# Britefury/cutmix-semisup-seg

Hardware: AMD Instinct MI355X
Metric: train images/sec (student+teacher step) (higher is better)
Workload: dtype bf16; 1 GPU; deeplab2-resnet101 cutmix mean-teacher step, 10x3x321x321, 21 classes (BASELINE configs[1]); per_gpu_batch=10, global_batch=10, classes=21, parallelism=dp1, fuse_batches=True, stream_overlap=True, deterministic_wgrad=False

## Files before the change

cutmix-semisup-seg_amd/_lib.py:

```python
import ctypes as C
import os

import torch

_HERE = os.path.dirname(os.path.abspath(__file__))
LIB_PATH = os.path.join(_HERE, 'csrc', 'libcutmixseg_hip.so')

if not os.path.exists(LIB_PATH):
    raise ImportError('libcutmixseg_hip.so not found at {} -- build it with '
                      '`python cutmix-semisup-seg_amd/build.py` (hipcc, gfx950); there is no CPU fallback'.format(LIB_PATH))

lib = C.CDLL(LIB_PATH)

F32, BF16 = 0, 1
(BN_REDUCE, BN_FINALIZE, BN_APPLY, BN_REDUCE_BWD, BN_BWD_APPLY, BN_COUNT, BN_STATS, BN_FINALIZE_TILES,
 BN_BWD_SUMS_TILES) = range(9)
LABEL_U8, LABEL_I64 = 0, 1
LOSS_IDS = {'var': 0, 'logits_var': 1, 'logits_smoothl1': 2, 'bce': 3, 'kld': 4}
MODE_MIX, MODE_CUT = 0, 1
OPT_CHUNK = 2048
AUG_PARAMS = 24

c_void_p, c_int, c_float, c_size_t = C.c_void_p, C.c_int, C.c_float, C.c_size_t

# ... 78 lines not shown


class StageEntry(C.Structure):
    _fields_ = [('img_off', C.c_longlong), ('lab_off', C.c_longlong), ('hs', c_int), ('ws', c_int)]


class StageDesc(C.Structure):
    _fields_ = [('pool_img', c_void_p), ('pool_labels', c_void_p), ('entries', c_void_p), ('index', c_void_p),
                ('out0', c_void_p), ('out1', c_void_p), ('out_labels', c_void_p), ('out_mask', c_void_p), ('params', c_void_p),
                ('mean', c_float * 3), ('std_', c_float * 3),
                ('n', c_int), ('n_entries', c_int), ('h', c_int), ('w', c_int), ('out_dtype', c_int)]


class PdPatch(C.Structure):
    _fields_ = [('img_off', C.c_longlong), ('hs', c_int), ('ws', c_int), ('cy', c_int), ('cx', c_int)]


class PackItem(C.Structure):
    _fields_ = [('src', c_void_p), ('dst', c_void_p), ('scale', c_void_p),
                ('ntaps', c_int), ('cout', c_int), ('cin', c_int), ('first_block', c_int)]


class WfinishItem(C.Structure):
    _fields_ = [('scratch', c_void_p), ('grad', c_void_p), ('w', c_void_p), ('scale', c_void_p), ('wdot', c_void_p),
                ('ntaps', c_int), ('cout', c_int), ('cin', c_int), ('first_block', c_int)]


_P = C.POINTER


def _proto(name, restype, argtypes):
    fn = getattr(lib, name)
    fn.restype = restype
    fn.argtypes = argtypes
    return fn


PROTOTYPES = {
    'cms_version': (c_int, []),
    'cms_last_error': (C.c_char_p, []),
    'cms_device_info': (c_int, [_P(c_int), C.c_char_p, c_size_t]),
    'cms_boxmask_rasterize': (c_int, [c_void_p, c_int, c_int, c_int, c_int, c_int, c_void_p, c_void_p]),
    'cms_cutmix_paste': (c_int, [c_void_p, c_void_p, c_void_p, c_int, c_void_p, c_int, c_int, c_int, c_int, c_int,
                                 c_int, c_void_p]),
    'cms_cutmix_paste_mask': (c_int, [c_void_p, c_void_p, c_void_p, c_int, c_void_p, c_int, c_int, c_int, c_int,
                                      c_void_p]),
    'cms_consistency_workspace_bytes': (c_size_t, [_P(ConsistencyDesc)]),
    'cms_consistency_fwd': (c_int, [_P(ConsistencyDesc), c_void_p, c_void_p, c_void_p]),
    'cms_consistency_finalize': (c_int, [c_void_p, c_void_p, c_float, c_int, c_float, c_float, c_void_p, c_void_p]),
    'cms_consistency_bwd': (c_int, [_P(ConsistencyDesc), c_void_p, c_void_p, c_void_p]),
    'cms_consistency_fused_supported': (c_int, [_P(ConsistencyDesc)]),
    'cms_consistency_fwd_bwd': (c_int, [_P(ConsistencyDesc), c_float, c_void_p, c_void_p, c_void_p, c_void_p]),
    'cms_scale_by_scalar': (c_int, [c_void_p, C.c_longlong, c_void_p, c_int, c_float, c_void_p]),
    'cms_ict_blend': (c_int, [c_void_p, c_void_p, c_void_p, c_int, c_void_p, c_int, C.c_longlong, c_void_p]),
    'cms_ict_workspace_bytes': (c_size_t, [_P(IctDesc)]),
    'cms_ict_fwd': (c_int, [_P(IctDesc), c_void_p, c_void_p, c_void_p]),
    'cms_ict_bwd': (c_int, [_P(IctDesc), c_void_p, c_void_p, c_void_p, c_void_p]),
    'cms_aug_workspace_bytes': (c_size_t, [_P(AugDesc)]),
    'cms_aug_fwd': (c_int, [_P(AugDesc), c_void_p, c_void_p, c_void_p]),
    'cms_aug_bwd': (c_int, [_P(AugDesc), c_void_p, c_void_p, c_void_p]),
    'cms_ce_workspace_bytes': (c_size_t, [_P(CeDesc)]),
    'cms_ce_fwd': (c_int, [_P(CeDesc), c_void_p, c_void_p, c_void_p]),
    'cms_ce_finalize': (c_int, [c_void_p, c_float, c_void_p, c_void_p]),
    'cms_ce_bwd': (c_int, [_P(CeDesc), c_void_p, c_void_p, c_void_p]),
    'cms_ce_fused_supported': (c_int, [_P(CeDesc)]),
    'cms_ce_fwd_bwd': (c_int, [_P(CeDesc), c_void_p, c_void_p, c_void_p, c_void_p]),
    'cms_upsample_bilinear_fwd': (c_int, [c_void_p, c_void_p, c_int, c_int, c_int, c_int, c_int, c_int, c_int,
                                          c_void_p]),
    'cms_upsample_bilinear_bwd': (c_int, [c_void_p, c_void_p, c_int, c_int, c_int, c_int, c_int, c_int, c_int,
                                          c_void_p]),
    'cms_ema_flat': (c_int, [c_void_p, c_void_p, c_size_t, c_float, c_float, c_void_p, c_void_p]),
    'cms_adam_ema_step': (c_int, [_P(OptimDesc), c_void_p]),
    'cms_sgd_ema_step': (c_int, [_P(OptimDesc), c_void_p]),
    'cms_increment_counter': (c_int, [c_void_p, c_void_p]),
    'cms_bn_fold': (c_int, [c_void_p, c_void_p, c_void_p, c_void_p, c_void_p, c_int, c_float, c_void_p, c_void_p, c_void_p]),
    'cms_argmax_confusion': (c_int, [c_void_p, c_void_p, c_int, c_int, c_int, c_int, c_int, c_int, c_int, c_int,
                                     c_int, c_void_p, c_void_p, c_void_p]),
    'cms_confusion': (c_int, [c_void_p, c_void_p, c_size_t, c_int, c_int, c_void_p, c_void_p]),
    'cms_fill_holes_workspace_bytes': (c_size_t, [c_int, c_int, c_int]),
    'cms_fill_holes': (c_int, [c_void_p, c_void_p, c_void_p, c_int, c_void_p, c_int, c_int, c_int, c_void_p, c_size_t,
                               c_void_p]),
    'cms_conv_igemm': (c_int, [_P(ConvDesc), c_void_p]),
    'cms_conv_igemm_workspace_bytes': (C.c_longlong, []),
    'cms_conv_igemm_route': (c_int, [_P(ConvDesc)]),
    'cms_conv_igemm_stats_tile_rows': (c_int, [_P(ConvDesc)]),
    'cms_frozen_bn_act_bwd': (c_int, [c_void_p, c_void_p, c_void_p, c_void_p, c_int, c_void_p, c_size_t, c_int, c_void_p]),
    'cms_conv_set_trace': (c_int, [c_void_p, c_int]),
    'cms_conv_set_wgrad8': (c_int, [c_int]),
    'cms_loss_set_deterministic': (c_int, [c_int]),
    'cms_conv_wgrad_uses_wgrad8': (c_int, [_P(WgradDesc)]),
    'cms_conv_wgrad': (c_int, [_P(WgradDesc), c_void_p]),
    'cms_conv_wgrad_workspace_bytes': (C.c_longlong, [_P(WgradDesc)]),
    'cms_conv_wgrad_group_kind': (c_int, [_P(WgradDesc)]),
    'cms_conv_wgrad_group_bytes': (C.c_longlong, [c_int]),
    'cms_conv_wgrad_group_pack': (c_int, [_P(WgradDesc), c_int, c_int, c_void_p, C.c_longlong, _P(c_int)]),
    'cms_conv_wgrad_group_run': (c_int, [c_void_p, c_int, c_int, c_int, c_void_p]),
    'cms_conv_pack_transpose': (c_int, [c_void_p, c_int, c_void_p, c_void_p, c_int, c_int, c_int, c_int, c_void_p]),
    'cms_conv_pack_transpose_batch': (c_int, [c_void_p, c_int, c_int, c_int, c_void_p]),
    'cms_conv_pack_transpose_batch64': (c_int, [c_void_p, c_int, c_int, c_void_p]),
    'cms_augment_batch': (c_int, [_P(AugmentDesc), c_void_p]),
    'cms_augment_luma': (c_int, [_P(AugmentDesc), c_void_p, c_void_p]),
    'cms_stage_batch': (c_int, [_P(StageDesc), c_void_p]),
    'cms_stage_luma': (c_int, [_P(StageDesc), c_void_p, c_void_p]),
    'cms_bn_workspace_bytes': (c_size_t, [c_size_t, c_int, c_int]),
    'cms_bn_run': (c_int, [_P(BnOp), c_void_p]),
    'cms_channel_copy': (c_int, [c_void_p, c_size_t, c_void_p, c_size_t, c_size_t, c_int, c_int, c_size_t, c_void_p]),
    'cms_add_n': (c_int, [c_void_p, c_int, c_void_p, c_size_t, c_int, c_void_p]),
    'cms_channel_sum': (c_int, [c_void_p, c_int, c_size_t, c_int, c_void_p, c_void_p]),
    'cms_wgrad_finish_pack': (c_int, [_P(WfinishItem), c_int]),
    'cms_wgrad_finish_run': (c_int, [c_void_p, c_int, c_int, c_void_p]),
    'cms_program_add_channel_sum': (c_int, [c_void_p, c_void_p, c_int, c_size_t, c_int, c_void_p, c_int, c_int]),
    'cms_program_add_wgrad_finish': (c_int, [c_void_p, c_void_p, c_int, c_int, c_int, c_int]),
    'cms_rows_reduce': (c_int, [c_void_p, c_size_t, c_int, c_size_t, c_int, c_int, c_void_p, c_float, c_void_p]),
    'cms_upsample_nhwc': (c_int, [c_void_p, c_void_p, c_size_t, c_int, c_int, c_int, c_int, c_int, c_int, c_int, c_int, c_int,
                                  c_void_p]),
    'cms_aspp_gather_fwd': (c_int, [c_void_p, c_void_p, c_void_p, _P(c_int), _P(c_int), c_int, c_int, c_int, c_int, c_int,
                                    c_int, c_void_p]),
    'cms_aspp_spread_bwd': (c_int, [c_void_p, c_void_p, c_int, _P(c_int), _P(c_int), c_int, c_int, c_int, c_int, c_int,
                                    c_int, c_void_p]),
    'cms_stem_pack_weights': (c_int, [c_void_p, c_int, c_void_p, c_void_p]),
    'cms_stem_out_hw': (c_int, [c_int, c_int, _P(c_int), _P(c_int), _P(c_int), _P(c_int)]),
    'cms_stem_fwd': (c_int, [c_void_p, c_int, c_void_p, c_int, c_void_p, c_void_p, c_void_p, c_int, c_int, c_int,
                             c_void_p]),
    'cms_maxpool3x3s2_fwd': (c_int, [c_void_p, c_void_p, c_void_p, c_int, c_int, c_int, c_int, c_int, c_int, c_void_p]),
    'cms_maxpool3x3s2_relu_bwd': (c_int, [c_void_p, c_void_p, c_void_p, c_void_p, c_int, c_int, c_int, c_int, c_int,
                                          c_int, c_void_p]),
    'cms_stem_wgrad': (c_int, [c_void_p, c_int, c_void_p, c_int, c_void_p, c_void_p, c_int, c_int, c_int, c_void_p]),
    'cms_stem_wgrad_workspace_bytes': (C.c_longlong, [c_int, c_int, c_int, c_int, c_int]),
    'cms_stem_wgrad_ws': (c_int, [c_void_p, c_int, c_void_p, c_int, c_void_p, c_void_p, c_int, c_int, c_int, c_void_p,
                          C.c_longlong, c_void_p]),
    'cms_stem_dgrad': (c_int, [c_void_p, c_int, c_void_p, c_void_p, c_void_p, c_int, c_int, c_int, c_void_p]),
    'cms_program_create': (c_int, [_P(c_void_p)]),
    'cms_program_destroy': (c_int, [c_void_p]),
    'cms_program_add_conv': (c_int, [c_void_p, _P(ConvDesc), c_int, c_int, c_int]),
    'cms_program_add_wgrad': (c_int, [c_void_p, _P(WgradDesc), c_int, c_int, c_int]),
    'cms_program_add_wgrad_group': (c_int, [c_void_p, c_void_p, c_int, c_int, c_int, c_int, c_int]),
    'cms_program_add_memset': (c_int, [c_void_p, c_void_p, c_size_t, c_int, c_int]),
    'cms_program_add_sync': (c_int, [c_void_p, c_int, c_int, c_int]),
    'cms_program_sync_count': (c_int, [c_void_p]),
    'cms_program_set_sync_flags': (c_int, [c_void_p, c_void_p, c_int]),
    'cms_program_add_aspp_gather': (c_int, [c_void_p, c_void_p, c_void_p, c_void_p, _P(c_int), _P(c_int), c_int, c_int,
                                            c_int, c_int, c_int, c_int, c_int, c_int]),
    'cms_program_add_aspp_spread': (c_int, [c_void_p, c_void_p, c_void_p, c_int, _P(c_int), _P(c_int), c_int, c_int, c_int,
                                            c_int, c_int, c_int, c_int, c_int]),
    'cms_program_add_bn': (c_int, [c_void_p, _P(BnOp), c_int, c_int]),
    'cms_program_size': (c_int, [c_void_p]),
    'cms_program_run': (c_int, [c_void_p, c_int, c_int, _P(c_void_p), c_int]),
    'cms_program_run_pair': (c_int, [c_void_p, _P(c_void_p), c_int, c_void_p, _P(c_void_p), c_int]),
    'cms_program_set_timing': (c_int, [c_void_p, c_int]),
    'cms_program_read_timing': (c_int, [c_void_p, _P(C.c_double), _P(C.c_double), _P(C.c_long), _P(C.c_double),
                                        _P(C.c_long)]),
    'cms_conv_igemm_f32': (c_int, [_P(ConvDesc), c_void_p]),
    'cms_conv_wgrad_f32': (c_int, [_P(WgradDesc), c_void_p]),
    'cms_conv_pack_transpose_f32': (c_int, [c_void_p, c_void_p, c_void_p, c_int, c_int, c_int, c_int, c_void_p]),
    'cms_conv_pack_transpose_batch_f32': (c_int, [c_void_p, c_int, c_int, c_void_p]),
    'cms_fft2': (c_int, [c_void_p, c_int, c_int, c_int, c_int, c_void_p, c_void_p, c_void_p]),
    'cms_pd_load_image': (c_int, [c_void_p, _P(StageEntry), c_int, c_int, c_int, c_int, c_void_p, c_void_p, c_void_p]),
    'cms_pd_load_patches': (c_int, [c_void_p, c_void_p, c_int, c_int, c_int, c_int, c_int, c_void_p, c_void_p]),
    'cms_pd_patch_sqdiff': (c_int, [c_void_p, c_void_p, c_void_p, c_int, c_int, c_int, c_void_p, c_void_p]),
    'cms_pd_spectrum_product': (c_int, [c_void_p, c_void_p, c_int, c_int, c_int, c_void_p, c_void_p]),
    'cms_pd_finish': (c_int, [c_void_p, c_void_p, c_void_p, c_int, c_int, c_int, c_int, c_int, c_void_p, c_void_p, c_void_p,
                              c_void_p]),
    'cms_select_workspace_bytes': (c_size_t, [c_int]),
    'cms_select_k_smallest': (c_int, [c_void_p, c_void_p, c_void_p, c_void_p, c_int, c_int, C.c_longlong, c_int, c_void_p, c_void_p,
                                      c_void_p, c_size_t, c_void_p]),
    'cms_pd_box_sum': (c_int, [c_void_p, c_int, c_int, c_int, c_int, c_int, c_void_p, c_void_p, c_void_p]),
    'cms_pd_neighbour_workspace_bytes': (c_size_t, [c_int, c_int, c_int, c_int]),
    'cms_pd_neighbour_maps': (c_int, [c_void_p, _P(StageEntry), c_int, c_int, c_void_p, c_void_p, c_void_p]),
    'cms_downsample_image_u8': (c_int, [c_void_p, c_int, c_int, c_int, c_int, c_void_p, c_void_p]),
    'cms_downsample_labels_u8': (c_int, [c_void_p, c_int, c_int, c_int, c_int, c_void_p, c_void_p]),
    'cms_cowmask_workspace_bytes': (c_size_t, [c_int, c_int, c_int]),
    'cms_cowmask': (c_int, [c_void_p, c_void_p, c_void_p, c_int, c_int, c_int, c_int, c_void_p, c_void_p, c_void_p, c_size_t,
                            c_void_p]),
}

fn = {}
for _name, (_res, _args) in PROTOTYPES.items():
    fn[_name] = _proto(_name, _res, _args)


class CmsError(RuntimeError):
    pass


def check(rc, what=''):
    if rc == 0:
        return
    msg = fn['cms_last_error']().decode(errors='replace')
    if rc == -1:
        raise ValueError('{}: {}'.format(what or 'cutmixseg', msg))
    raise CmsError('{} failed (code {}): {}'.format(what or 'cutmixseg', rc, msg))


def version():
    return fn['cms_version']()
```

cutmix-semisup-seg_amd/backbone_hip.py:

```python
import os
import torch

from . import ops
from .arena import ensure_arena


def executors_of(module):
    exs = getattr(module, '_hip_executors', None)
    if exs:
        return list(exs.values())
    ex = getattr(module, '_hip_executor', None)
    return [] if ex is None else [ex]


class _Conv(object):
    __slots__ = ('wkey', 'bn', 'taps', 'ntaps', 'neg_taps', 'stride', 'cin', 'cout', 'scale', 'bias', 'wT', 'ksize',
                 'pad', 'dil', 'wdot', 'dbeta', 'wT_raw')

    def __init__(self, wkey, bn, conv):
        self.wkey, self.bn = wkey, bn
        kh, kw = conv.kernel_size
        self.ksize, self.pad, self.dil = kh, conv.padding[0], conv.dilation[0]
        self.taps = ops.conv_taps(kh, kw, conv.dilation[0], conv.padding[0])
        self.neg_taps = [(-dy, -dx) for dy, dx in self.taps]
# ... 13 lines not shown
        self._init_common(net, dtype)
        self.num_classes = net.num_classes
        self._add_blocks('', [getattr(net, 'layer{}'.format(li)) for li in range(1, 5)])
        self.stem_wkey, self.stem_bn, self.stem_ceil = 'conv1.weight', 'bn1', True
        self.stem_w147 = None
        self._stem_version = -1
        head = net.layer5.conv2d_list
        self.aspp_keys = ['layer5.conv2d_list.0', 'layer5.conv2d_list.1']
        self.aspp_taps = []
        for i in range(2):
            self.aspp_taps += ops.conv_taps(3, 3, head[i].dilation[0], head[i].padding[0])
        self.aspp_neg_taps = [(-dy, -dx) for dy, dx in self.aspp_taps]
        dev = self.arena.device
        C = self.num_classes
        if C > 32:
            raise NotImplementedError('ASPP head kernel is specialised for <= 32 classes')
        self.aspp_zc = (18 * C + 127) // 128 * 128
        self.aspp_wall = torch.zeros(1, self.aspp_zc, 2048, dtype=self.dtype, device=dev)
        self.aspp_wallT = torch.zeros(1, 2048, self.aspp_zc, dtype=self.dtype, device=dev)
        self._aspp_version = -1
        self.aspp_bias = torch.zeros(C, dtype=torch.float32, device=dev)

    def _init_common(self, net, dtype=torch.bfloat16):
        if dtype not in (torch.bfloat16, torch.float32):
            raise TypeError('executor dtype must be torch.bfloat16 or torch.float32')
        self.net = net
        self.dtype = dtype
        self.trainable = any(p.requires_grad for p in net.parameters())
        self.bn_trainable = any(p.requires_grad for m in net.modules() if 'BatchNorm' in type(m).__name__
                                for p in m.parameters())
        self.arena = ensure_arena(net, with_grad=self.trainable, with_bf16=(dtype == torch.bfloat16))
        self.blocks = []
        self._layer_first = []
        self._affine_ready = False
        self._bn_idx = None
        self._side = None
        self._pack_plan = None
        self._pack_plan_bn = None
        self._wT_raw_version = -1
        self._bn_modules = {}
        self._stem_param = None
        self._sentinel = None
        self._seen_shapes = {}
        self._wscratch_buf = None
        self._wfinish_pending = []
        self._wfinish_ok = {}
        self._pending_keep = None
        self.grad_hook = None
        self.data_grad_only = False
        self.overlap_wgrad = True
        self.wgrad_streams = 2 if os.environ.get('CMS_WGRAD8', '1') != '0' else 1
        self.defer_wgrad_join = False
        self._pending_join = None
        self._sides = []
        self.conv_tile = 0
        self.tile_rules = {}
        self._wT_version = -1
        self.version = 0
        self.use_programs = True
        self._programs = {}
        self._generation = 0
        self.issued = dict(flops=0.0, conv_launches=0, conv_bytes=0.0, head_launches=0, head_bytes=0.0, head_bytes_alg=0.0, floor_s=0.0)
        net.register_load_state_dict_post_hook(lambda module, incompatible: self.invalidate())

    def _add_blocks(self, prefix, layers):
        for li, layer in enumerate(layers):
            self._layer_first.append(len(self.blocks))
            for bi, blk in enumerate(layer):
                pre = '{}layer{}.{}'.format(prefix, li + 1, bi)
                b = _Block()
                b.c1 = _Conv(pre + '.conv1.weight', pre + '.bn1', blk.conv1)
                b.c2 = _Conv(pre + '.conv2.weight', pre + '.bn2', blk.conv2)
                b.c3 = _Conv(pre + '.conv3.weight', pre + '.bn3', blk.conv3)
                b.cd = None
                if blk.downsample is not None:
                    b.cd = _Conv(pre + '.downsample.0.weight', pre + '.downsample.1', blk.downsample[0])
                self.blocks.append(b)

    def invalidate(self):
        self.arena.refresh_bf16()
        self._affine_ready = False
        self.version += 1

    def weights_changed(self, bn_too=False):
        self.version += 1
        if bn_too or self.bn_trainable:
            self._affine_ready = False

    def block_grad_offsets(self):
        return [self.arena.by_key[b.c1.wkey].offset for b in self.blocks]

    def layer_first_blocks(self):
        return list(self._layer_first)

    def _all_convs(self):
        for b in self.blocks:
            for c in (b.c1, b.c2, b.c3, b.cd):
                if c is not None:
                    yield c

    def _build_affine_tables(self):
        a = self.arena
        idx = {k: [] for k in ('weight', 'bias', 'running_mean', 'running_var')}
        off = 0
        spans = []
        for c in self._all_convs():
# ... 193 lines not shown
            ops.bn_op('sums_tiles', c=C, dtype=self.dtype, n_pixels=npix, groups=G, tile_rows=tile_stats['tile_rows'],
                      ws=tile_stats['tile_sums'], sums=sums)
        else:
            ops.bn_op('reduce_bwd', c=C, dtype=self.dtype, n_pixels=npix, groups=G, x=u, dy=dy, mean=mean, rstd=rstd, sums=sums,
                      ws=ws, mask_bits=bits)
        grp = self._dist_group()
        world = ops._world(grp)
        if world > 1:
            ops.host_call(lambda t=sums, g_=grp: ops._allreduce_sum(t, g_))
        du = torch.empty_like(u)
        dres = torch.empty_like(u) if want_res else None
        ops.bn_op('bwd_apply', c=C, dtype=self.dtype, n_pixels=npix, groups=G, count=(npix // G) * world, x=u, dy=dy, dx=du, dres=dres,
                  mask_bits=bits, mean=mean, rstd=rstd, gamma=self.arena.view(c.bn + '.weight'), sums=sums)
        return du, dres

    def _fwd_block_bn(self, st, bi):
        b, cur = self.blocks[bi], st['cur']
        save, G = st['saved'] is not None, st.get('groups', 1)
        a1, s1 = self._fwd_unit_bn(cur, b.c1, True, save=save, groups=G)
        a2, s2 = self._fwd_unit_bn(a1, b.c2, True, save=save, groups=G)
        sd = None
        if b.cd is None:
            res = cur
        else:
            res, sd = self._fwd_unit_bn(cur, b.cd, False, save=save, groups=G)
        out, s3 = self._fwd_unit_bn(a2, b.c3, True, res=res, save=save, groups=G)
        st['cur'] = out
        if st['saved'] is not None:
            st['saved'].append((cur, a1, a2, s1, s2, s3, sd))

    def _refresh_backward_weights_bn(self):
        if self._pack_plan_bn is None:
            triples = []
            for c in self._all_convs():
                w = self._w(c)
                c.wT_raw = torch.empty((w.shape[0], w.shape[2], w.shape[1]), dtype=self.dtype, device=w.device)
                triples.append((w, c.wT_raw, None))
            triples.append((self.aspp_wall, self.aspp_wallT, None))
            self._pack_plan_bn = ops.PackTransposePlan(triples)
        self._pack_plan_bn.run()

    def _dgrad_raw(self, du, c, res=None, in_hw=None, res_bits=None, bstats=None):
        n, ho, wo, _ = du.shape
        if c.stride == 1:
            return ops.conv_igemm(du, c.wT_raw, c.neg_taps, res=res, mode=1, tile=self._tile(c.cin), mask_bits=res_bits,
                                  mask_gates_res=res_bits is not None, stats=bstats)
        assert res_bits is None and bstats is None
        return ops.conv_igemm(du, c.wT_raw, c.neg_taps, res=res, mode=1, out_hw=(ho, wo), out_stride=c.stride,
                              out_full_hw=in_hw, tile=self._tile(c.cin))

    def _wgrad_raw(self, du, x, c):
        ops.conv_wgrad(du, x, c.taps, self.arena.packed(c.wkey, self.arena.grad), stride=c.stride, wg_target=self._wg_target())

    def _backward_chain_bn(self, saved, dlg, want_w, sides, hook, box=None):
        x4 = saved[-1]
        main = torch.cuda.current_stream()
        d = ops.aspp_spread_bwd(dlg, self.aspp_taps, self.aspp_zc, self.dtype)
        dwall = None
        if want_w:
            dwall = torch.empty((1, self.aspp_zc, 2048), dtype=torch.float32, device=d.device)
            ops.memset_zero(dwall)
            ops.conv_wgrad(d, x4, [(0, 0)], dwall)
            if box is not None:
                box['dwall'] = dwall
        pend = self._bstats(saved[len(self.blocks) - 1][5])
        dOut = ops.conv_igemm(d, self.aspp_wallT, [(0, 0)], mode=1, stats=pend)
        keep = []
        closes = set(self.bucket_starts())
        for bi in range(len(self.blocks) - 1, -1, -1):
            b = self.blocks[bi]
            xin, a1, a2, s1, s2, s3, sd = saved[bi]
            in_hw = (xin.shape[1], xin.shape[2])
            bits3 = s3[1] if (b.cd is not None or (b.c1.stride == 1 and self.dtype == torch.bfloat16)) else None
            du3, dres = self._bwd_unit_bn(dOut, s3, b.c3, bits3 is None, tile_stats=pend)
            da2 = self._dgrad_raw(du3, b.c3)
            du2, _ = self._bwd_unit_bn(da2, s2, b.c2, False)
            da1 = self._dgrad_raw(du2, b.c2)
            du1, _ = self._bwd_unit_bn(da1, s1, b.c1, False)
            dud = None
            if b.cd is not None:
                dud, _ = self._bwd_unit_bn(dres if bits3 is None else dOut, sd, b.cd, False, dy_bits=bits3)
            if want_w:
                self._issue_wgrads(self._block_jobs(b, du3, du2, dud, du1, xin, a1, a2), sides, main, keep, bi in closes,
                                   wgrad=self._wgrad_raw)
                with torch.cuda.stream(sides[0] if sides else main):
                    hook(bi)
            pend = self._bstats(saved[bi - 1][5]) if (bi > 0 and b.c1.stride == 1) else None
            if b.cd is None and bits3 is not None:
                dOut = self._dgrad_raw(du1, b.c1, res=dOut, in_hw=in_hw, res_bits=bits3, bstats=pend)
            else:
                dx = dres if b.cd is None else self._dgrad_raw(dud, b.cd, in_hw=in_hw)
                dOut = self._dgrad_raw(du1, b.c1, res=dx, in_hw=in_hw, bstats=pend)
        if not self.defer_wgrad_join:
            for sd_ in sides:
                ops.stream_wait(main, sd_)
        self._retire_keep(keep)
        return dOut, dwall

    def _stem_prepare(self):
        if not self._affine_ready:
            self._refresh_affine()
        if self._stem_version != self.version:
            self.stem_w147 = ops.stem_pack_weights(self.arena.packed(self.stem_wkey, self._wbuf()), out=self.stem_w147)
            self._stem_version = self.version

    def stem(self, x):
        if self._stem_param is None:
            self._stem_param = dict(self.net.named_parameters())[self.stem_wkey]
        save = (torch.is_grad_enabled() and (self.trainable or x.requires_grad)) if self.use_programs else None
        return _StemFn.apply(x.contiguous(), self._stem_param, self, save)
# ... 130 lines not shown
    def _wscratch(self):
        if self._wscratch_buf is None:
            self._wscratch_buf = torch.zeros_like(self.arena.grad)
        return self._wscratch_buf

    def _wfinish_takes(self, du, x, c):
        if self.dtype != torch.bfloat16 or ops.deterministic_wgrad():
            return False
        key = (c.wkey, tuple(du.shape), tuple(x.shape))
        hit = self._wfinish_ok.get(key)
        if hit is None:
            hit = self._wfinish_ok[key] = bool(ops.conv_wgrad(du, x, c.taps, self.arena.packed(c.wkey, self._wscratch()),
                                                              stride=c.stride, scale=None, wg_target=self._wg_target(),
                                                              query_kernel=True))
        return hit

    def _wfinish_flush(self):
        pend = self._wfinish_pending
        if not pend:
            return
        a = self.arena
        ops.wgrad_finish([(a.packed(c.wkey, self._wscratch()), a.packed(c.wkey, a.grad), self._w(c), c.scale, c.wdot) for c in pend])
        del pend[:]

    def _wg_target(self):
        if not self.overlap_wgrad:
            return 0
        return 56 if self.wgrad_streams >= 2 else 112

    def _dgrad(self, du, c, res=None, mask=None, in_hw=None):
        n, ho, wo, _ = du.shape
        mb = getattr(mask, '_cms_relu_bits', None) if mask is not None else None
        if mb is not None:
            mask = None
        if c.stride == 1:
            return ops.conv_igemm(du, c.wT, c.neg_taps, res=res, mode=1, mask_src=mask, tile=self._tile(c.cin), mask_bits=mb)
        return ops.conv_igemm(du, c.wT, c.neg_taps, res=res, mode=1, mask_src=mask, out_hw=(ho, wo),
                              out_stride=c.stride, out_full_hw=in_hw, tile=self._tile(c.cin), mask_bits=mb)

    def _grad_sentinel(self):
        if self._sentinel is None:
            self._sentinel = dict(self.net.named_parameters())[self.blocks[-1].c3.wkey]
        return self._sentinel

    def _want_w(self):
        data_only = self.data_grad_only or getattr(self.net, '_data_grad_only', False)
        return self.trainable and not data_only and self.arena.grad is not None

    def _refresh_for_backward(self):
        if self._wT_version != self.version or self.blocks[0].c1.wT is None:
            self._refresh_backward_weights()
            self._wT_version = self.version

    def _head_bias_grads(self, dlogits, want_w, side=None):
        if want_w:
            if side is not None:
                side.wait_stream(torch.cuda.current_stream())
                dlogits.record_stream(side)
            with torch.cuda.stream(side if side is not None else torch.cuda.current_stream()):
                db = dlogits.sum(dim=(0, 2, 3))
                for k in self.aspp_keys:
                    self.arena.view(k + '.bias', self.arena.grad).add_(db)

    def _head_weight_grads(self, dwall, side=None):
        C = self.num_classes
        a = self.arena
        with torch.cuda.stream(side if side is not None else torch.cuda.current_stream()):
            for i, k in enumerate(self.aspp_keys):
                a.packed(k + '.weight', a.grad).add_(dwall[0, 9 * C * i:9 * C * (i + 1)].view(9, C, 2048))

    def _finish_head(self, dwall, side):
        self._head_weight_grads(dwall, side)
        if side is not None and not self.defer_wgrad_join:
            torch.cuda.current_stream().wait_stream(side)

    def bucket_starts(self):
        l2, l3, l4 = self._layer_first[1], self._layer_first[2], self._layer_first[3]
        return sorted(set([0, l2, l3, (l3 + l4 + 1) // 2, l4]))

    def _backward_chain(self, saved, dlg, want_w, sides, hook, box=None):
        x4 = saved[-1]
        main = torch.cuda.current_stream()
        d = ops.aspp_spread_bwd(dlg, self.aspp_taps, self.aspp_zc, self.dtype)
        dwall = None
        keep = []
        if want_w:
            dwall = torch.empty((1, self.aspp_zc, 2048), dtype=torch.float32, device=d.device)
            hs = sides[0] if sides else None
            if hs is not None:
                ops.stream_wait(hs, main)
                keep.append((d, dwall))
            with torch.cuda.stream(hs if hs is not None else main):
                ops.memset_zero(dwall)
                ops.conv_wgrad(d, x4, [(0, 0)], dwall)
            if box is not None:
                box['dwall'] = dwall
        x4b = getattr(x4, '_cms_relu_bits', None)
        dC = ops.conv_igemm(d, self.aspp_wallT, [(0, 0)], mode=1, mask_src=None if x4b is not None else x4, mask_bits=x4b)
        capture = getattr(self, 'debug_capture', None)
        closes = set(self.bucket_starts())
        for bi in range(len(self.blocks) - 1, -1, -1):
            if capture is not None:
                capture[bi] = dC
            b = self.blocks[bi]
            xin, a1, a2 = saved[bi]
            in_hw = (xin.shape[1], xin.shape[2])
            dU2 = self._dgrad(dC, b.c3, mask=a2)
            dU1 = self._dgrad(dU2, b.c2, mask=a1)
            if want_w:
                self._issue_wgrads(self._block_jobs(b, dC, dU2, dC, dU1, xin, a1, a2), sides, main, keep, bi in closes)
                with torch.cuda.stream(sides[0] if sides else main):
                    hook(bi)
            dres = dC if b.cd is None else self._dgrad(dC, b.cd, in_hw=in_hw)
            dC = self._dgrad(dU1, b.c1, res=dres, mask=None if bi == 0 else xin, in_hw=in_hw)
        if not self.defer_wgrad_join:
            for sd in sides:
                ops.stream_wait(main, sd)
        self._retire_keep(keep)
        return dC, dwall

    def backward(self, token, dlogits):
        bn = (token[0].bn if self.use_programs and isinstance(token, tuple) and isinstance(token[0], ops.Program)
              else len(token[0]) == 7)
        chain = self._backward_chain_bn if bn else self._backward_chain
        if bn:
            if self._wT_raw_version != self.version or self.blocks[0].c1.wT_raw is None:
                self._refresh_aspp_fwd()
                self._refresh_backward_weights_bn()
                self._wT_raw_version = self.version
        else:
            self._refresh_for_backward()
        want_w = self._want_w()
        if want_w and self._grad_sentinel().grad is None:
            self.arena.ensure_grads_attached()
        n, _, h, w = dlogits.shape
        main = torch.cuda.current_stream()
        sides = self._side_streams(self.wgrad_streams) if (self.overlap_wgrad and want_w) else []
        hside = sides[0] if (sides and not bn) else None
        if not self.use_programs:
            if self.defer_wgrad_join and sides:
                self._pending_join = list(sides)
            self._head_bias_grads(dlogits, want_w, hside)
            box = {}

            def hook(bi):
                if 'done' not in box and box.get('dwall') is not None:
                    self._head_weight_grads(box['dwall'])
                    box['done'] = True
                if self.grad_hook is not None:
                    self.grad_hook(bi)
            dx, dwall = chain(token, dlogits, want_w, sides, hook, box)
            if dwall is not None and 'done' not in box:
                self._finish_head(dwall, hside)
            return dx
        fprog, gen = token
        if fprog.generation != gen:
            raise RuntimeError('the activations of this forward pass were overwritten by a later forward pass of the '
                               'same shape through the same executor (programs keep ONE set of buffers per shape): '
                               'run backward before the next forward, or set executor.use_programs = False')
        key = (want_w, len(sides), bool(self.defer_wgrad_join))
        if self.defer_wgrad_join and sides:
            self._pending_join = list(sides)
        prog = fprog.bwd.get(key)
        if prog is None:
            prog = ops.Program()
            dlg = torch.empty(tuple(dlogits.shape), dtype=torch.float32, device=dlogits.device)
            streams = [main] + sides
            with ops.recording(prog, streams):
                dx, dwall = chain(fprog.saved, dlg, want_w, sides, prog.mark)
            prog.dlg, prog.dx, prog.dwall = dlg, dx, dwall
            fprog.bwd[key] = prog
        prog.dlg.copy_(dlogits)
        self._head_bias_grads(dlogits, want_w, hside)
        streams = [main] + sides
        if self.grad_hook is None or not want_w:
            prog.run(streams)
            if prog.dwall is not None:
                self._finish_head(prog.dwall, hside)
        else:
            first = 0
            hook_stream = sides[0] if sides else main
            head_done = False
            wanted = getattr(self.grad_hook, 'blocks', None)
            for idx, bi in prog.marks:
                if wanted is not None and bi not in wanted:
                    continue
                prog.run(streams, first, idx)
                first = idx
                with torch.cuda.stream(hook_stream):
                    if not head_done and prog.dwall is not None:
                        self._head_weight_grads(prog.dwall)
                        head_done = True
                    self.grad_hook(bi)
            prog.run(streams, first, -1)
            if prog.dwall is not None and not head_done:
                self._finish_head(prog.dwall, hside)
        self._account(prog)
        return prog.dx.clone()

    def _retire_keep(self, keep):
        if keep and self.defer_wgrad_join and ops._REC is None:
            self._pending_keep = (self._pending_keep or []) + [keep]

    def join_wgrad(self):
        sides, self._pending_join = self._pending_join, None
        if sides:
            main = torch.cuda.current_stream()
            for sd in sides:
                main.wait_stream(sd)
        self._pending_keep = None

    @staticmethod
    def _block_jobs(b, d3, d2, dd, d1, xin, a1, a2):
        return [(d3, a2, b.c3), (d2, a1, b.c2)] + ([(dd, xin, b.cd)] if b.cd is not None else []) + [(d1, xin, b.c1)]

    def _issue_wgrads(self, jobs, sides, main, keep, closes, first=0, wgrad=None):
        wgrad = wgrad or self._wgrad
        for sd in sides:
            ops.stream_wait(sd, main)
        if sides:
            keep.append(jobs)
        for ji, (du_, x_, c_) in enumerate(jobs, first):
            with torch.cuda.stream(sides[ji % len(sides)] if sides else main):
                wgrad(du_, x_, c_)
        if closes:
            for sd in sides[1:]:
# ... 479 lines not shown
        logits, token = executor.forward(x_nhwc, save=need_grad)
        ctx.executor = executor
        ctx.saved_acts = token
        return logits

    @staticmethod
    def backward(ctx, dlogits):
        dx = ctx.executor.backward(ctx.saved_acts, dlogits.contiguous().float())
        ctx.saved_acts = None
        return dx, None, None


class _BodyPairFn(torch.autograd.Function):

    @staticmethod
    def forward(ctx, x_stu, x_tea, ex_stu, ex_tea, side, need_grad):
        if ex_stu.use_programs and ex_tea.use_programs:
            main = torch.cuda.current_stream()
            ps = ex_stu.forward_program(x_stu.shape, need_grad)
            ex_stu._prepare_forward()
            if x_stu.data_ptr() != ps.x_in.data_ptr():
                ps.x_in.copy_(x_stu)
            with torch.cuda.stream(side):
                pt = ex_tea.forward_program(x_tea.shape, False)
                ex_tea._prepare_forward()
                if x_tea.data_ptr() != pt.x_in.data_ptr():
                    pt.x_in.copy_(x_tea)
            if ps.host_ops or pt.host_ops:
                with torch.cuda.stream(side):
                    pt.run([side])
                ps.run([main])
            else:
                ops.run_pair(ps, [main], pt, [side])
            ex_stu._stamp(ps)
            ex_tea._stamp(pt)
            logits_s = ps.logits.clone()
            with torch.cuda.stream(side):
                logits_t = pt.logits.clone()
            saved = (ps, ps.generation) if need_grad else None
        else:
            st_s = ex_stu.fwd_begin(x_stu, need_grad)
            with torch.cuda.stream(side):
                st_t = ex_tea.fwd_begin(x_tea, False)
            for bi in range(len(ex_stu.blocks)):
                ex_stu.fwd_block(st_s, bi)
                with torch.cuda.stream(side):
                    ex_tea.fwd_block(st_t, bi)
            logits_s, saved = ex_stu.fwd_end(st_s)
            with torch.cuda.stream(side):
                logits_t, _ = ex_tea.fwd_end(st_t)
        ctx.executor = ex_stu
        ctx.saved_acts = saved
        ctx.mark_non_differentiable(logits_t)
        return logits_s, logits_t

    @staticmethod
    def backward(ctx, dlogits, _unused):
        dx = ctx.executor.backward(ctx.saved_acts, dlogits.contiguous().float())
        ctx.saved_acts = None
        return dx, None, None, None, None, None


def run_body_pair(ex_stu, x_stu, ex_tea, x_tea, side):
    if len(ex_stu.blocks) != len(ex_tea.blocks):
        raise ValueError('student and teacher bodies differ')
    need_grad = torch.is_grad_enabled() and ex_stu.trainable
    if need_grad and not x_stu.requires_grad:
        x_stu = x_stu.detach().requires_grad_(True)
    return _BodyPairFn.apply(x_stu, x_tea, ex_stu, ex_tea, side, need_grad)


def run_body(executor, x_nhwc):
    need_grad = torch.is_grad_enabled() and (executor.trainable or x_nhwc.requires_grad)
    if need_grad and not x_nhwc.requires_grad:
        x_nhwc = x_nhwc.detach().requires_grad_(True)
    return _BodyFn.apply(x_nhwc, executor, need_grad)
```

cutmix-semisup-seg_amd/csrc/aspp.hip:

```cpp
#include "common.hpp"

namespace cms {

struct AsppTaps {
    int n_taps;
    short dy[CMS_CONV_MAX_TAPS], dx[CMS_CONV_MAX_TAPS];
};

__device__ __forceinline__ void taps_to_lds(const AsppTaps& tp, short* sdy, short* sdx) {
#pragma unroll
    for (int i = 0; i < CMS_CONV_MAX_TAPS; ++i)
        if ((int)threadIdx.x == i) {
            sdy[i] = tp.dy[i];
            sdx[i] = tp.dx[i];
        }
    __syncthreads();
}

__global__ __launch_bounds__(256) void aspp_gather_fwd_kernel(const float* __restrict__ z, const float* __restrict__ bias,
                                                              float* __restrict__ logits, AsppTaps tp, int N, int C, int ZC,
                                                              int H, int W) {
    __shared__ short sdy[CMS_CONV_MAX_TAPS], sdx[CMS_CONV_MAX_TAPS];
    taps_to_lds(tp, sdy, sdx);
    const int n_taps = tp.n_taps;
    const size_t total = (size_t)N * C * H * W;
    for (size_t i = (size_t)blockIdx.x * blockDim.x + threadIdx.x; i < total; i += (size_t)gridDim.x * blockDim.x) {
        const unsigned ii = (unsigned)i;
        const int x = (int)(ii % (unsigned)W);
        unsigned t = ii / (unsigned)W;
        const int y = (int)(t % (unsigned)H); t /= (unsigned)H;
        const int c = (int)(t % (unsigned)C);
        const int n = (int)(t / (unsigned)C);
        float acc = bias ? bias[c] : 0.0f;
        const float* zn = z + ((size_t)n * ZC + c) * H * W;
        const size_t tap_stride = (size_t)C * H * W;
        for (int k = 0; k < n_taps; ++k) {
            const int yy = y + sdy[k], xx = x + sdx[k];
            if ((unsigned)yy < (unsigned)H && (unsigned)xx < (unsigned)W) acc += zn[(size_t)k * tap_stride + (size_t)yy * W + xx];
        }
        logits[i] = acc;
    }
}

template <class T>
__global__ __launch_bounds__(256) void aspp_spread_bwd_kernel(const float* __restrict__ dl, T* __restrict__ d, AsppTaps tp,
                                                              int N, int C, int ZC, int H, int W) {
    __shared__ short sdy[CMS_CONV_MAX_TAPS], sdx[CMS_CONV_MAX_TAPS];
    taps_to_lds(tp, sdy, sdx);
    const int n_taps = tp.n_taps;
    const unsigned zc8 = (unsigned)ZC / 8u;
    const size_t total = (size_t)N * H * W * zc8;
    const size_t plane = (size_t)H * W;
    for (size_t i = (size_t)blockIdx.x * blockDim.x + threadIdx.x; i < total; i += (size_t)gridDim.x * blockDim.x) {
        const unsigned ii = (unsigned)i;
        const unsigned ch = ii % zc8;
        unsigned t = ii / zc8;
        const int x = (int)(t % (unsigned)W); t /= (unsigned)W;
        const int y = (int)(t % (unsigned)H);
        const int n = (int)(t / (unsigned)H);
        const float* dn = dl + (size_t)n * C * plane;
        float v[8];
        int k = (int)((ch * 8u) / (unsigned)C), c = (int)(ch * 8u) - k * C;
#pragma unroll
        for (int e = 0; e < 8; ++e) {
            float val = 0.0f;
            if (k < n_taps) {
                const int yy = y - sdy[k], xx = x - sdx[k];
                if ((unsigned)yy < (unsigned)H && (unsigned)xx < (unsigned)W) val = dn[(size_t)c * plane + (size_t)yy * W + xx];
            }
            v[e] = val;
            if (++c == C) { c = 0; ++k; }
        }
        if constexpr (sizeof(T) == 4) {
            float4* o = reinterpret_cast<float4*>(d + i * 8);
            o[0] = float4{v[0], v[1], v[2], v[3]};
            o[1] = float4{v[4], v[5], v[6], v[7]};
        } else {
            uint4 o;
            o.x = (uint32_t)f32_to_bf16(v[0]) | ((uint32_t)f32_to_bf16(v[1]) << 16);
            o.y = (uint32_t)f32_to_bf16(v[2]) | ((uint32_t)f32_to_bf16(v[3]) << 16);
            o.z = (uint32_t)f32_to_bf16(v[4]) | ((uint32_t)f32_to_bf16(v[5]) << 16);
            o.w = (uint32_t)f32_to_bf16(v[6]) | ((uint32_t)f32_to_bf16(v[7]) << 16);
            *reinterpret_cast<uint4*>(d + i * 8) = o;
        }
    }
}

}

using namespace cms;

static int fill_taps(AsppTaps& tp, const int* dy, const int* dx, int n_taps) {
    CMS_REQUIRE(dy && dx && n_taps > 0 && n_taps <= CMS_CONV_MAX_TAPS, "aspp: 1..%d taps", CMS_CONV_MAX_TAPS);
    tp.n_taps = n_taps;
    for (int i = 0; i < CMS_CONV_MAX_TAPS; ++i) {
        tp.dy[i] = (short)(i < n_taps ? dy[i] : 0);
        tp.dx[i] = (short)(i < n_taps ? dx[i] : 0);
    }
    return CMS_OK;
}

extern "C" int cms_aspp_gather_fwd(const float* z, const float* bias, float* logits, const int* tap_dy, const int* tap_dx,
                                   int n_taps, int n, int c, int zc, int h, int w, void* stream) {
    CMS_REQUIRE(z && logits, "aspp_gather_fwd: NULL pointer");
    CMS_REQUIRE(n > 0 && c > 0 && h > 0 && w > 0 && zc >= n_taps * c, "aspp_gather_fwd: bad geometry (zc >= taps * classes)");
    AsppTaps tp;
    const int rc = fill_taps(tp, tap_dy, tap_dx, n_taps);
    if (rc) return rc;
    const size_t total = (size_t)n * c * h * w;
    CMS_REQUIRE(total < (1ull << 32), "aspp_gather_fwd: more than 2^32 logits");
    hipLaunchKernelGGL(aspp_gather_fwd_kernel, dim3(grid_for(total, 256, 256 * 16)), dim3(256), 0, (hipStream_t)stream, z, bias,
                       logits, tp, n, c, zc, h, w);
    return launch_status("cms_aspp_gather_fwd");
}

extern "C" int cms_aspp_spread_bwd(const float* dlogits, void* d_nhwc, int d_dtype, const int* tap_dy, const int* tap_dx,
                                   int n_taps, int n, int c, int zc, int h, int w, void* stream) {
    CMS_REQUIRE(dlogits && d_nhwc, "aspp_spread_bwd: NULL pointer");
    CMS_REQUIRE(d_dtype == CMS_F32 || d_dtype == CMS_BF16, "aspp_spread_bwd: bad dtype");
    CMS_REQUIRE(n > 0 && c > 0 && h > 0 && w > 0 && zc >= n_taps * c, "aspp_spread_bwd: bad geometry (zc >= taps * classes)");
    AsppTaps tp;
    const int rc = fill_taps(tp, tap_dy, tap_dx, n_taps);
    if (rc) return rc;
    CMS_REQUIRE(zc % 8 == 0, "aspp_spread_bwd: the stacked tap x class axis (%d) must be a multiple of 8", zc);
    const size_t total = (size_t)n * h * w * (zc / 8);
    CMS_REQUIRE(total < (1ull << 32), "aspp_spread_bwd: more than 2^32 chunks");
    hipStream_t s = (hipStream_t)stream;
    if (d_dtype == CMS_F32)
        hipLaunchKernelGGL(aspp_spread_bwd_kernel<float>, dim3(grid_for(total, 256, 256 * 16)), dim3(256), 0, s, dlogits,
                           (float*)d_nhwc, tp, n, c, zc, h, w);
    else
        hipLaunchKernelGGL(aspp_spread_bwd_kernel<uint16_t>, dim3(grid_for(total, 256, 256 * 16)), dim3(256), 0, s, dlogits,
                           (uint16_t*)d_nhwc, tp, n, c, zc, h, w);
    return launch_status("cms_aspp_spread_bwd");
}
```

cutmix-semisup-seg_amd/csrc/loss_tiles.hpp:

```cpp
#pragma once
#include <algorithm>
#include <cstdlib>
#include "common.hpp"

namespace cms {

template <bool IDENT>
struct Gather {
    const float* base;
    size_t plane;
    int w_in;
    Tap ty, tx;
    size_t off;
    __device__ __forceinline__ float operator()(int c) const {
        if (IDENT) return base[c * plane + off];
        return bilin_gather(base + c * plane, w_in, ty, tx);
    }
};

template <int CT>
struct RegVec {
    float v[CT > 0 ? CT : 1];
    __device__ __forceinline__ float operator()(int c) const { return v[c]; }
};
// ... 123 lines not shown
    const int ty_i = b % tiles_y;
    ScatterTile t;
    t.n = b / tiles_y;
    t.x0 = tx_i * TILE_W;
    t.y0 = ty_i * FWD_TILE_H;
    t.tw = min(TILE_W, g.W - t.x0);
    t.th = min(FWD_TILE_H, g.H - t.y0);
    return t;
}

template <bool UNROLL, class Stage, class Pixel>
__device__ __forceinline__ void fwd_tile_walk(const Geo& g, float* smem, Stage stage, Pixel pixel) {
    const ScatterTile t = fwd_tile(g);
    const Patch p = tile_patch(g, t.x0, t.y0, t.tw, t.th);
    stage(t.n, p, smem);
    __syncthreads();
    const int col = threadIdx.x & (TILE_W - 1);
    auto rows = [&](int rr) {
        const int row = (threadIdx.x >> 6) + rr * 4;
        if (col < t.tw && row < t.th) {
            const int y = t.y0 + row, x = t.x0 + col;
            Tap ty = bilin_tap(y, g.sy, g.h, g.align != 0), tx = bilin_tap(x, g.sx, g.w, g.align != 0);
            rebase(ty, tx, p);
            pixel(t.n, y, x, ty, tx, p);
        }
    };
    if (UNROLL) {
#pragma unroll
        for (int rr = 0; rr < FWD_TILE_H / 4; ++rr) rows(rr);
    } else {
#pragma unroll 1
        for (int rr = 0; rr < FWD_TILE_H / 4; ++rr) rows(rr);
    }
}

template <class F>
__device__ __forceinline__ void pixel_walk(const Geo& g, F f) {
    const size_t P = (size_t)g.n * g.H * g.W;
    for (size_t idx = (size_t)blockIdx.x * blockDim.x + threadIdx.x; idx < P; idx += (size_t)gridDim.x * blockDim.x) {
        const int x = (int)(idx % g.W);
        const size_t t = idx / g.W;
        const int y = (int)(t % g.H);
        const int n = (int)(t / g.H);
        f(idx, n, y, x);
    }
}

template <int K>
__device__ __forceinline__ void store_partials(float (&acc)[K], float* red, float* __restrict__ partials) {
    block_sum<K>(acc, red);
    if (threadIdx.x == 0) {
#pragma unroll
        for (int k = 0; k < K; ++k) partials[blockIdx.x * K + k] = acc[k];
    }
}

template <int K>
__global__ __launch_bounds__(256) void reduce_partials_kernel(const float* __restrict__ partials, int nblocks,
                                                              double* __restrict__ out, double extra, int extra_slot) {
    __shared__ double sm[K][256];
    double loc[K];
#pragma unroll
    for (int k = 0; k < K; ++k) loc[k] = 0.0;
    for (int i = threadIdx.x; i < nblocks; i += 256) {
#pragma unroll
        for (int k = 0; k < K; ++k) loc[k] += (double)partials[i * K + k];
    }
#pragma unroll
    for (int k = 0; k < K; ++k) sm[k][threadIdx.x] = loc[k];
    __syncthreads();
    for (int s = 128; s > 0; s >>= 1) {
        if ((int)threadIdx.x < s) {
#pragma unroll
            for (int k = 0; k < K; ++k) sm[k][threadIdx.x] += sm[k][threadIdx.x + s];
        }
        __syncthreads();
    }
    if (threadIdx.x == 0) {
#pragma unroll
        for (int k = 0; k < K; ++k) out[k] = sm[k][0];
        if (extra_slot >= 0) out[extra_slot] = extra;
    }
}

#ifndef CMS_LOSS_TILE_H
#define CMS_LOSS_TILE_H 4
#endif
constexpr int TILE_H = CMS_LOSS_TILE_H;
constexpr int G_LD = TILE_W + 1;

struct TileTables {
    int xi0[TILE_W], xi1[TILE_W];
    float xw1[TILE_W];
    int yi0[TILE_H], yi1[TILE_H];
    float yw1[TILE_H];
    int xbeg[TILE_W + 2], xend[TILE_W + 2];
};

inline int tile_max_rows(float sy) { return tile_max_rows_of(sy, TILE_H); }

inline size_t tile_lds_bytes(int C, float sy, float sx, int n_patches) {
    size_t g = (size_t)TILE_H * C * G_LD;
    size_t r = (size_t)TILE_H * C * tile_max_cols(sx);
    return (g + r + (size_t)n_patches * patch_floats(C, sy, sx, TILE_H)) * sizeof(float);
}

// ... 253 lines not shown
```

cutmix-semisup-seg_amd/csrc/losses.hip:

```cpp
#include "loss_tiles.hpp"

namespace cms {

struct ConsArgs {
    cms_consistency_desc d;
    Geo g;
    float tau, inv_root_c;
};

struct ConsPixel {
    bool m;
    float um;
    const float* tea;
    int which;
};

__device__ __forceinline__ ConsPixel cons_pixel_inputs(const ConsArgs& a, int n, int y, int x) {
    const cms_consistency_desc& d = a.d;
    const size_t pix = ((size_t)n * d.H + y) * d.W + x;
    ConsPixel p;
    if (d.mask) {
        p.m = d.mask[pix] >= 0.5f;
    } else {
        p.m = box_mask_bit(d.ranges + (size_t)n * d.n_boxes * 4, d.n_boxes, y, x, d.invert != 0);
// ... 21 lines not shown
}

template <int CT, bool IDENT>
__device__ __forceinline__ void cons_fwd_pixel(const ConsArgs& a, const ConsPixel& px, const Gather<IDENT>& gs, const Gather<IDENT>& gt,
                                               float (&acc)[3]) {
    const Geo& g = a.g;
    PixelFwd r;
    if (CT > 0) {
        RegVec<CT> rs, rt;
        fill<CT, IDENT>(rs, gs);
        fill<CT, IDENT>(rt, gt);
        r = consistency_pixel_fwd<CT>(rs, rt, g.c, a.d.loss_fn, a.inv_root_c);
    } else {
        r = consistency_pixel_fwd<0>(gs, gt, g.c, a.d.loss_fn, a.inv_root_c);
    }
    const float lm = r.loss * px.um;
    const float cf = (a.tau > 0.0f && r.conf >= a.tau) ? 1.0f : 0.0f;
    acc[0] += lm;
    acc[1] += lm * cf;
    acc[2] += cf;
}

template <int CT>
__global__ __launch_bounds__(256) void cons_fwd_tiled_kernel(ConsArgs a, float* __restrict__ partials, int patch_stride) {
    extern __shared__ __attribute__((aligned(16))) float smem[];
    float acc[3] = {0.0f, 0.0f, 0.0f};
    fwd_tile_walk<false>(
        a.g, smem, [&](int n, const Patch& p, float* P) { cons_stage(a, n, p, P, patch_stride); },
        [&](int n, int y, int x, const Tap& ty, const Tap& tx, const Patch& p) {
            const ConsPixel px = cons_pixel_inputs(a, n, y, x);
            const Gather<false> gs = gather_staged(smem, p, ty, tx);
            const Gather<false> gt = gather_staged(smem + (px.which ? 2 : 1) * patch_stride, p, ty, tx);
            cons_fwd_pixel<CT, false>(a, px, gs, gt, acc);
        });
    __shared__ float red[3 * 16];
    store_partials<3>(acc, red, partials);
}

template <int CT, bool IDENT>
__global__ __launch_bounds__(256) void cons_fwd_kernel(ConsArgs a, float* __restrict__ partials) {
    const Geo& g = a.g;
    float acc[3] = {0.0f, 0.0f, 0.0f};
    pixel_walk(g, [&](size_t, int n, int y, int x) {
        const ConsPixel px = cons_pixel_inputs(a, n, y, x);
        const Gather<IDENT> gs = gather_at<IDENT>(a.d.l_stu + (size_t)n * g.c * ((size_t)g.h * g.w), g, y, x);
        Gather<IDENT> gt = gs;
        gt.base = px.tea;
        cons_fwd_pixel<CT, IDENT>(a, px, gs, gt, acc);
    });
    __shared__ float red[3 * 16];
    store_partials<3>(acc, red, partials);
}

__global__ void cons_finalize_kernel(const double* __restrict__ sl, const double* __restrict__ sg, float tau,
                                     int per_pixel, float ramp, float weight, float* __restrict__ out) {
    if (threadIdx.x != 0 || blockIdx.x != 0) return;
    const double Pl = sl[3];
    double closs, gs, rate;
    if (tau > 0.0f) {
        rate = sg[2] / sg[3];
        if (per_pixel) {
            closs = sl[1] / Pl;
            gs = 1.0 / Pl;
        } else {
            closs = rate * (sl[0] / Pl);
            gs = rate / Pl;
        }
    } else {
        rate = NAN;
        closs = sl[0] / Pl;
        gs = 1.0 / Pl;
    }
    closs *= (double)ramp;
    out[0] = (float)closs;
    out[1] = (float)rate;
    out[2] = (float)(gs * (double)ramp * (double)weight);
    out[3] = (float)(closs * (double)weight);
}

template <int CT>
__global__ __launch_bounds__(256) void cons_bwd_ident_kernel(ConsArgs a, const float* __restrict__ scalars,
                                                             float* __restrict__ grad) {
    const Geo& g = a.g;
    const size_t plane = (size_t)g.h * g.w;
    const float gscale = scalars[2];
    pixel_walk(g, [&](size_t, int n, int y, int x) {
        const ConsPixel px = cons_pixel_inputs(a, n, y, x);
        const Gather<true> gs = gather_at<true>(a.d.l_stu + (size_t)n * g.c * plane, g, y, x);
        Gather<true> gt = gs;
        gt.base = px.tea;
        float* gp = grad + (size_t)n * g.c * plane + gs.off;
        const float base_f = gscale * px.um;
        const bool pp = a.tau > 0.0f && a.d.conf_per_pixel;
        if (CT > 0) {
            RegVec<CT> rs, rt;
            fill<CT, true>(rs, gs);
            fill<CT, true>(rt, gt);
            float gv[CT > 0 ? CT : 1];
            const float conf = consistency_pixel_bwd<CT>(rs, rt, g.c, a.d.loss_fn, a.inv_root_c,
                                                        [&](int k, float v) { gv[k] = v; });
            const float f = (pp && !(conf >= a.tau)) ? 0.0f : base_f;
#pragma unroll
            for (int k = 0; k < CT; ++k) gp[k * plane] += f * gv[k];
        } else {
            float ms, zs, mt, zt;
            softmax_stats<0>(gt, g.c, mt, zt);
            (void)ms; (void)zs;
            const float conf = 1.0f / zt;
            const float f = (pp && !(conf >= a.tau)) ? 0.0f : base_f;
            consistency_pixel_bwd<0>(gs, gt, g.c, a.d.loss_fn, a.inv_root_c,
                                     [&](int k, float v) { gp[k * plane] += f * v; });
        }
    });
}

template <int CT>
__global__ __launch_bounds__(256) void cons_bwd_tiled_kernel(ConsArgs a, const float* __restrict__ scalars,
                                                             float* __restrict__ grad, int patch_stride) {
    extern __shared__ __attribute__((aligned(16))) float smem[];
    const Geo& g = a.g;
    const float gscale = scalars[2];
    const bool pp = a.tau > 0.0f && a.d.conf_per_pixel;
    const int pstride = patch_stride;
    auto stage = [&](int n, const Patch& p, float* P) { cons_stage(a, n, p, P, pstride); };
    auto pixel_grad = [&](int n, int y, int x, const Tap& ty, const Tap& tx, const Patch& p, const float* P, auto emit) -> bool {
        const ConsPixel px = cons_pixel_inputs(a, n, y, x);
        const float base_f = gscale * px.um;
        const Gather<false> gs = gather_staged(P, p, ty, tx);
        const Gather<false> gt = gather_staged(P + (px.which ? 2 * pstride : pstride), p, ty, tx);
        if (CT > 0) {
            RegVec<CT> rs, rt;
            fill<CT, false>(rs, gs);
            fill<CT, false>(rt, gt);
            float gv[CT > 0 ? CT : 1];
            const float conf = consistency_pixel_bwd<CT>(rs, rt, g.c, a.d.loss_fn, a.inv_root_c,
                                                        [&](int k, float v) { gv[k] = v; });
            const float f = (pp && !(conf >= a.tau)) ? 0.0f : base_f;
#pragma unroll
            for (int k = 0; k < CT; ++k) emit(k, f * gv[k]);
        } else {
            float mt, zt;
            softmax_stats<0>(gt, g.c, mt, zt);
            const float conf = 1.0f / zt;
            const float f = (pp && !(conf >= a.tau)) ? 0.0f : base_f;
            consistency_pixel_bwd<0>(gs, gt, g.c, a.d.loss_fn, a.inv_root_c, [&](int k, float v) { emit(k, f * v); });
        }
        return true;
    };
    tiled_scatter(g, stage, pixel_grad, grad, smem);
}

template <int CT, int LF>
__global__ __launch_bounds__(256, (LF >= 0 && CT > 0) ? 4 : 1) void cons_fused_tiled_kernel(ConsArgs a, float grad_unit, float* __restrict__ grad,
                                                               int patch_stride, float* __restrict__ partials) {
    extern __shared__ __attribute__((aligned(16))) float smem[];
    const Geo& g = a.g;
    const bool pp = a.tau > 0.0f && a.d.conf_per_pixel;
    const int pstride = patch_stride;
    float acc[3] = {0.0f, 0.0f, 0.0f};
    auto stage = [&](int n, const Patch& p, float* P) { cons_stage(a, n, p, P, pstride); };
    auto pixel_grad = [&](int n, int y, int x, const Tap& ty, const Tap& tx, const Patch& p, const float* P, auto emit) -> bool {
        const ConsPixel px = cons_pixel_inputs(a, n, y, x);
        const float base_f = grad_unit * px.um;
        const Gather<false> gs = gather_staged(P, p, ty, tx);
        const Gather<false> gt = gather_staged(P + (px.which ? 2 * pstride : pstride), p, ty, tx);
        PixelFwd r;
        if (CT > 0) {
            RegVec<CT> rs, rt;
            fill<CT, false>(rs, gs);
            fill<CT, false>(rt, gt);
            r = consistency_pixel_fwd_bwd<(CT > 0 ? CT : 1), LF>(
                rs, rt, a.d.loss_fn, a.inv_root_c,
                [&](float conf) -> float { return (pp && !(conf >= a.tau)) ? 0.0f : base_f; },
                [&](int k, float v) { emit(k, v); });
        } else {
            r = consistency_pixel_fwd<0>(gs, gt, g.c, a.d.loss_fn, a.inv_root_c);
            const float f = (pp && !(r.conf >= a.tau)) ? 0.0f : base_f;
            consistency_pixel_bwd<0>(gs, gt, g.c, a.d.loss_fn, a.inv_root_c, [&](int k, float v) { emit(k, f * v); });
        }
        const float lm = r.loss * px.um;
        const float cf = (a.tau > 0.0f && r.conf >= a.tau) ? 1.0f : 0.0f;
        acc[0] += lm;
        acc[1] += lm * cf;
        acc[2] += cf;
        return true;
    };
    tiled_scatter(g, stage, pixel_grad, grad, smem);
    __shared__ float red[3 * 16];
    store_partials<3>(acc, red, partials);
}

__global__ __launch_bounds__(256) void scale_by_scalar_kernel(float* __restrict__ x, size_t n, const float* __restrict__ scalars,
                                                              int idx, float factor) {
    const float f = scalars[idx] * factor;
    for (size_t i = (size_t)blockIdx.x * blockDim.x + threadIdx.x; i < n; i += (size_t)gridDim.x * blockDim.x) x[i] *= f;
}

struct CeArgs {
    cms_ce_desc d;
    Geo g;
};

__device__ __forceinline__ int load_label(const CeArgs& a, size_t pix) {
    if (a.d.label_dtype == CMS_LABEL_U8) return (int)((const uint8_t*)a.d.labels)[pix];
    const int64_t v = ((const int64_t*)a.d.labels)[pix];
    return (v < 0 || v > 0x7fffffff) ? -1 : (int)v;
}

__device__ __forceinline__ bool ce_ignored(const CeArgs& a, int label) {
    return label == a.d.ignore_index || label < 0 || label >= a.g.c;
}

__device__ __forceinline__ void ce_stage(const CeArgs& a, int n, const Patch& p, float* P) {
    const Geo& g = a.g;
    const size_t plane = (size_t)g.h * g.w;
    stage_patch(P, a.d.logits + (size_t)n * g.c * plane, g.c, plane, g.w, p);
}

template <int CT, bool IDENT>
__device__ __forceinline__ void ce_fwd_pixel(const CeArgs& a, const Gather<IDENT>& gl, int label, float (&acc)[2]) {
    float v;
    if (CT > 0) {
        RegVec<CT> r;
        fill<CT, IDENT>(r, gl);
        float mx, z;
        softmax_stats<CT>(r, a.g.c, mx, z);
        v = -((gl(label) - mx) - logf(z));
    } else {
        v = ce_pixel_fwd<0>(gl, a.g.c, label);
    }
    acc[0] += v;
    acc[1] += 1.0f;
}

template <int CT, bool IDENT>
__global__ __launch_bounds__(256) void ce_fwd_kernel(CeArgs a, float* __restrict__ partials) {
    const Geo& g = a.g;
    float acc[2] = {0.0f, 0.0f};
    pixel_walk(g, [&](size_t pix, int n, int y, int x) {
        const int label = load_label(a, pix);
        if (ce_ignored(a, label)) return;
        ce_fwd_pixel<CT, IDENT>(a, gather_at<IDENT>(a.d.logits + (size_t)n * g.c * ((size_t)g.h * g.w), g, y, x), label, acc);
    });
    __shared__ float red[2 * 16];
    store_partials<2>(acc, red, partials);
}

template <int CT>
__global__ __launch_bounds__(256) void ce_fwd_tiled_kernel(CeArgs a, float* __restrict__ partials) {
    extern __shared__ __attribute__((aligned(16))) float smem[];
    const Geo& g = a.g;
    float acc[2] = {0.0f, 0.0f};
    fwd_tile_walk<true>(
        g, smem, [&](int n, const Patch& p, float* P) { ce_stage(a, n, p, P); },
        [&](int n, int y, int x, const Tap& ty, const Tap& tx, const Patch& p) {
            const int label = load_label(a, ((size_t)n * g.H + y) * g.W + x);
            if (ce_ignored(a, label)) return;
            ce_fwd_pixel<CT, false>(a, gather_staged(smem, p, ty, tx), label, acc);
        });
    __shared__ float red[2 * 16];
    store_partials<2>(acc, red, partials);
}

__global__ void ce_finalize_kernel(const double* __restrict__ stats, float weight, float* __restrict__ out) {
    if (threadIdx.x != 0 || blockIdx.x != 0) return;
    out[0] = (float)(stats[0] / stats[1]);
    out[1] = stats[1] > 0.0 ? (float)((double)weight / stats[1]) : 0.0f;
}

template <int CT>
__global__ __launch_bounds__(256) void ce_bwd_ident_kernel(CeArgs a, const float* __restrict__ scalars,
                                                           float* __restrict__ grad) {
    const Geo& g = a.g;
    const size_t plane = (size_t)g.h * g.w;
    const float gscale = scalars[1];
    pixel_walk(g, [&](size_t pix, int n, int y, int x) {
        const int label = load_label(a, pix);
        if (ce_ignored(a, label)) return;
        const Gather<true> gl = gather_at<true>(a.d.logits + (size_t)n * g.c * plane, g, y, x);
        float* gp = grad + (size_t)n * g.c * plane + gl.off;
        if (CT > 0) {
            RegVec<CT> r;
            fill<CT, true>(r, gl);
            ce_pixel_bwd<CT>(r, g.c, label, [&](int k, float v) { gp[k * plane] += gscale * v; });
        } else {
            ce_pixel_bwd<0>(gl, g.c, label, [&](int k, float v) { gp[k * plane] += gscale * v; });
        }
    });
}

template <int CT>
__global__ __launch_bounds__(256) void ce_bwd_tiled_kernel(CeArgs a, const float* __restrict__ scalars,
                                                           float* __restrict__ grad) {
    extern __shared__ __attribute__((aligned(16))) float smem[];
    const Geo& g = a.g;
    const float gscale = scalars[1];
    auto stage = [&](int n, const Patch& p, float* P) { ce_stage(a, n, p, P); };
    auto pixel_grad = [&](int n, int y, int x, const Tap& ty, const Tap& tx, const Patch& p, const float* P, auto emit) -> bool {
        const size_t pix = ((size_t)n * g.H + y) * g.W + x;
        const int label = load_label(a, pix);
        if (ce_ignored(a, label)) return false;
        const Gather<false> gl = gather_staged(P, p, ty, tx);
        if (CT > 0) {
            RegVec<CT> r;
            fill<CT, false>(r, gl);
            ce_pixel_bwd<CT>(r, g.c, label, [&](int k, float v) { emit(k, gscale * v); });
        } else {
            ce_pixel_bwd<0>(gl, g.c, label, [&](int k, float v) { emit(k, gscale * v); });
        }
        return true;
    };
    tiled_scatter(g, stage, pixel_grad, grad, smem);
}

template <int CT>
__global__ __launch_bounds__(256) void ce_fused_tiled_kernel(CeArgs a, float* __restrict__ grad, float* __restrict__ partials) {
    extern __shared__ __attribute__((aligned(16))) float smem[];
    const Geo& g = a.g;
    float acc[2] = {0.0f, 0.0f};
    auto stage = [&](int n, const Patch& p, float* P) { ce_stage(a, n, p, P); };
    auto pixel_grad = [&](int n, int y, int x, const Tap& ty, const Tap& tx, const Patch& p, const float* P, auto emit) -> bool {
        const size_t pix = ((size_t)n * g.H + y) * g.W + x;
        const int label = load_label(a, pix);
        if (ce_ignored(a, label)) return false;
        const Gather<false> gl = gather_staged(P, p, ty, tx);
        float v;
        if (CT > 0) {
            RegVec<CT> r;
            fill<CT, false>(r, gl);
            v = ce_pixel_fwd_bwd<(CT > 0 ? CT : 1)>(r, gl(label), label, [&](int k, float gv) { emit(k, gv); });
        } else {
            v = ce_pixel_fwd<0>(gl, g.c, label);
            ce_pixel_bwd<0>(gl, g.c, label, [&](int k, float gv) { emit(k, gv); });
        }
        acc[0] += v;
        acc[1] += 1.0f;
        return true;
    };
    tiled_scatter(g, stage, pixel_grad, grad, smem);
    __shared__ float red[2 * 16];
    store_partials<2>(acc, red, partials);
}

static int g_loss_deterministic = -1;
bool loss_deterministic() {
    if (g_loss_deterministic < 0) {
        const char* e = getenv("CMS_LOSS_DETERMINISTIC");
        g_loss_deterministic = e ? (atoi(e) != 0) : 0;
    }
    return g_loss_deterministic != 0;
}

int fwd_tiles(const Geo& g, int n_patches, size_t* lds_out, int* stride_out) {
    if (is_ident(g)) return 0;
    static int on = -1;
    if (on < 0) {
        const char* e = getenv("CMS_LOSS_FWD_TILED");
        on = e ? (atoi(e) != 0) : 1;
    }
    if (!on) return 0;
    const size_t pf = patch_floats(g.c, g.sy, g.sx, FWD_TILE_H);
    const size_t lds = pf * n_patches * sizeof(float);
    if (lds > FWD_PATCH_LDS_MAX) return 0;
    if (lds_out) *lds_out = lds;
    if (stride_out) *stride_out = (int)pf;
    return ((g.W + TILE_W - 1) / TILE_W) * ((g.H + FWD_TILE_H - 1) / FWD_TILE_H) * g.n;
}

int fused_tiles(const Geo& g, int n_patches) {
    if (is_ident(g)) return 0;
    if (loss_deterministic()) return 0;
    static int on = -1;
    if (on < 0) {
        const char* e = getenv("CMS_LOSS_FUSED");
        on = e ? (atoi(e) != 0) : 1;
    }
    if (!on) return 0;
    if (tile_lds_bytes(g.c, g.sy, g.sx, n_patches) > TILE_LDS_MAX) return 0;
    return ((g.W + TILE_W - 1) / TILE_W) * ((g.H + TILE_H - 1) / TILE_H) * g.n;
}

static int check_cons(const cms_consistency_desc* d) {
    CMS_REQUIRE(d != nullptr, "consistency: null descriptor");
    CMS_REQUIRE(d->l_stu && d->l_tea0, "consistency: l_stu / l_tea0 must not be NULL");
    CMS_REQUIRE(d->mode == CMS_MODE_MIX || d->mode == CMS_MODE_CUT, "consistency: unknown mode %d", d->mode);
    CMS_REQUIRE(d->mode != CMS_MODE_MIX || d->l_tea1, "consistency: mix mode needs l_tea1");
    CMS_REQUIRE((d->ranges != nullptr) != (d->mask != nullptr), "consistency: give exactly one of ranges / mask");
    CMS_REQUIRE(d->ranges == nullptr || d->n_boxes >= 0, "consistency: n_boxes < 0");
    int rc = check_geometry(d, "consistency");
    return rc ? rc : check_loss_fn(d);
}

static ConsArgs make_cons_args(const cms_consistency_desc* d) {
    ConsArgs a;
    a.d = *d;
    a.g = geo_of(d);
    a.tau = d->conf_thresh;
    a.inv_root_c = (float)(1.0 / sqrt((double)d->c));
    return a;
}

static int check_ce(const cms_ce_desc* d) {
    CMS_REQUIRE(d != nullptr, "ce: null descriptor");
    CMS_REQUIRE(d->logits && d->labels, "ce: logits / labels NULL");
    CMS_REQUIRE(d->label_dtype == CMS_LABEL_U8 || d->label_dtype == CMS_LABEL_I64, "ce: bad label dtype");
    return check_geometry(d, "ce", "label");
}

static CeArgs make_ce_args(const cms_ce_desc* d) {
    CeArgs a;
    a.d = *d;
    a.g = geo_of(d);
    return a;
}

template <int K, class Kern, class... Args>
static void launch_fused(Kern kern, int tiles, size_t lds, hipStream_t s, float* partials, double* stats_out, double extra, int extra_slot,
                         Args... args) {
    allow_lds(kern, lds);
    hipLaunchKernelGGL(kern, dim3(tiles), dim3(256), lds, s, args..., partials);
    hipLaunchKernelGGL((reduce_partials_kernel<K>), dim3(1), dim3(256), 0, s, partials, tiles, stats_out, extra, extra_slot);
}

}

using namespace cms;

extern "C" size_t cms_consistency_workspace_bytes(const cms_consistency_desc* d) {
    if (!d) return 0;
    const Geo g = geo_of(d);
    return (size_t)std::max(fwd_blocks(g, 3), fused_tiles(g, 3)) * 3 * sizeof(float);
}

extern "C" int cms_consistency_fused_supported(const cms_consistency_desc* d) {
    if (check_cons(d)) return 0;
    return fused_tiles(geo_of(d), 3) > 0 ? 1 : 0;
}

extern "C" int cms_consistency_fwd_bwd(const cms_consistency_desc* d, float grad_unit, void* workspace, double* stats_out,
                                       float* grad_l_stu, void* stream) {
    int rc = check_cons(d);
    if (rc) return rc;
    CMS_REQUIRE(workspace && stats_out && grad_l_stu, "consistency_fwd_bwd: workspace / stats_out / grad NULL");
    ConsArgs a = make_cons_args(d);
    const int tiles = fused_tiles(a.g, 3);
    CMS_REQUIRE(tiles > 0, "consistency_fwd_bwd: not available for this geometry / mode (ask cms_consistency_fused_supported)");
    hipStream_t s = (hipStream_t)stream;
    const int pstride = (int)patch_floats(d->c, a.g.sy, a.g.sx, TILE_H);
    CMS_DISPATCH_C(d->c, {
        auto kern = d->loss_fn == CMS_LOSS_VAR ? cons_fused_tiled_kernel<CT, LOSS_VAR> : cons_fused_tiled_kernel<CT, -1>;
        launch_fused<3>(kern, tiles, tile_lds_bytes(d->c, a.g.sy, a.g.sx, 3), s, (float*)workspace, stats_out,
                        (double)((size_t)d->n * d->H * d->W), 3, a, grad_unit, grad_l_stu, pstride);
    });
    return launch_status("cms_consistency_fwd_bwd");
}

extern "C" int cms_scale_by_scalar(float* x, long long n, const float* scalars, int index, float factor, void* stream) {
    CMS_REQUIRE(x && scalars && n >= 0 && index >= 0, "scale_by_scalar: bad argument");
    if (n == 0) return CMS_OK;
    const int grid = (int)std::min<long long>((n + 255) / 256, 1024);
    hipLaunchKernelGGL(scale_by_scalar_kernel, dim3(grid), dim3(256), 0, (hipStream_t)stream, x, (size_t)n, scalars, index, factor);
    return launch_status("cms_scale_by_scalar");
}

extern "C" int cms_consistency_fwd(const cms_consistency_desc* d, void* workspace, double* stats_out, void* stream) {
    int rc = check_cons(d);
    if (rc) return rc;
    CMS_REQUIRE(workspace && stats_out, "consistency_fwd: workspace / stats_out NULL");
    ConsArgs a = make_cons_args(d);
    const FwdPlan p = fwd_plan(a.g, 3);
    CMS_DISPATCH_C(d->c, launch_fwd<3>(cons_fwd_tiled_kernel<CT>, cons_fwd_kernel<CT, true>, cons_fwd_kernel<CT, false>, a, p,
                                       (float*)workspace, stats_out, (double)((size_t)d->n * d->H * d->W), 3,
                                       (hipStream_t)stream, p.pstride));
    return launch_status("cms_consistency_fwd");
}

extern "C" int cms_consistency_finalize(const double* stats_local, const double* stats_global, float conf_thresh,
                                        int conf_per_pixel, float ramp_val, float cons_weight, float* scalars_out,
                                        void* stream) {
    CMS_REQUIRE(stats_local && stats_global && scalars_out, "consistency_finalize: NULL argument");
    hipLaunchKernelGGL(cons_finalize_kernel, dim3(1), dim3(64), 0, (hipStream_t)stream, stats_local, stats_global,
                       conf_thresh, conf_per_pixel, ramp_val, cons_weight, scalars_out);
    return launch_status("cms_consistency_finalize");
}

extern "C" int cms_loss_set_deterministic(int on) {
    cms::g_loss_deterministic = on ? 1 : 0;
    return CMS_OK;
}

extern "C" int cms_consistency_bwd(const cms_consistency_desc* d, const float* scalars, float* grad_l_stu,
                                   void* stream) {
    int rc = check_cons(d);
    if (rc) return rc;
    CMS_REQUIRE(scalars && grad_l_stu, "consistency_bwd: scalars / grad NULL");
    ConsArgs a = make_cons_args(d);
    const int pstride = (int)patch_floats(d->c, a.g.sy, a.g.sx, TILE_H);
    CMS_DISPATCH_C(d->c, rc = launch_bwd("consistency_bwd", cons_bwd_ident_kernel<CT>, cons_bwd_tiled_kernel<CT>, a, 3, 0, scalars,
                                         grad_l_stu, (hipStream_t)stream, pstride));
    return rc ? rc : launch_status("cms_consistency_bwd");
}

extern "C" size_t cms_ce_workspace_bytes(const cms_ce_desc* d) {
    if (!d) return 0;
    const Geo g = geo_of(d);
    return (size_t)std::max(fwd_blocks(g, 1), fused_tiles(g, 1)) * 2 * sizeof(float);
}

extern "C" int cms_ce_fused_supported(const cms_ce_desc* d) {
    if (check_ce(d)) return 0;
    return fused_tiles(geo_of(d), 1) > 0 ? 1 : 0;
}

extern "C" int cms_ce_fwd_bwd(const cms_ce_desc* d, void* workspace, double* stats_out, float* grad_logits, void* stream) {
    int rc = check_ce(d);
    if (rc) return rc;
    CMS_REQUIRE(workspace && stats_out && grad_logits, "ce_fwd_bwd: workspace / stats_out / grad NULL");
    const CeArgs a = make_ce_args(d);
    const int tiles = fused_tiles(a.g, 1);
    CMS_REQUIRE(tiles > 0, "ce_fwd_bwd: not available for this geometry / mode (ask cms_ce_fused_supported)");
    CMS_DISPATCH_C(d->c, launch_fused<2>(ce_fused_tiled_kernel<CT>, tiles, tile_lds_bytes(d->c, a.g.sy, a.g.sx, 1), (hipStream_t)stream,
                                         (float*)workspace, stats_out, 0.0, -1, a, grad_logits));
    return launch_status("cms_ce_fwd_bwd");
}

extern "C" int cms_ce_fwd(const cms_ce_desc* d, void* workspace, double* stats_out, void* stream) {
    int rc = check_ce(d);
    if (rc) return rc;
    CMS_REQUIRE(workspace && stats_out, "ce_fwd: workspace / stats_out NULL");
    const CeArgs a = make_ce_args(d);
    const FwdPlan p = fwd_plan(a.g, 1);
    CMS_DISPATCH_C(d->c, launch_fwd<2>(ce_fwd_tiled_kernel<CT>, ce_fwd_kernel<CT, true>, ce_fwd_kernel<CT, false>, a, p,
                                       (float*)workspace, stats_out, 0.0, -1, (hipStream_t)stream));
    return launch_status("cms_ce_fwd");
}

extern "C" int cms_ce_finalize(const double* stats, float loss_weight, float* scalars_out, void* stream) {
    CMS_REQUIRE(stats && scalars_out, "ce_finalize: NULL argument");
    hipLaunchKernelGGL(ce_finalize_kernel, dim3(1), dim3(64), 0, (hipStream_t)stream, stats, loss_weight, scalars_out);
    return launch_status("cms_ce_finalize");
}

extern "C" int cms_ce_bwd(const cms_ce_desc* d, const float* scalars, float* grad_logits, void* stream) {
    int rc = check_ce(d);
    if (rc) return rc;
    CMS_REQUIRE(scalars && grad_logits, "ce_bwd: scalars / grad NULL");
    const CeArgs a = make_ce_args(d);
    CMS_DISPATCH_C(d->c, rc = launch_bwd("ce_bwd", ce_bwd_ident_kernel<CT>, ce_bwd_tiled_kernel<CT>, a, 1, 0, scalars, grad_logits,
                                         (hipStream_t)stream));
    return rc ? rc : launch_status("cms_ce_bwd");
}
```

cutmix-semisup-seg_amd/csrc/program.hip:

```cpp
#include <cstdlib>
#include "common.hpp"
#include <new>
#include <vector>

namespace cms {

enum OpKind { OP_CONV = 0, OP_WGRAD = 1, OP_MEMSET = 2, OP_SYNC = 3, OP_ASPP_GATHER = 4, OP_ASPP_SPREAD = 5, OP_BN = 6, OP_WGRAD_GROUP = 7, OP_CHANNEL_SUM = 8, OP_WGRAD_FINISH = 9 };

struct AsppOp {
    const float* src;
    const float* bias;
    void* dst;
    int d_dtype;
    int tap_dy[CMS_CONV_MAX_TAPS], tap_dx[CMS_CONV_MAX_TAPS];
    int n_taps, n, c, zc, h, w;
};

__global__ __launch_bounds__(64) void sync_set_kernel(int* flag, int v) {
    if (threadIdx.x == 0) __hip_atomic_store(flag, v, __ATOMIC_RELEASE, __HIP_MEMORY_SCOPE_AGENT);
}

__global__ __launch_bounds__(64) void sync_wait_kernel(const int* flag, int v, int* timeouts) {
    if (threadIdx.x != 0) return;
    const long long t0 = wall_clock64();
// ... 54 lines not shown

using namespace cms;

static int issue(cms_program* p, Op& o, void* const* streams, int n_streams) {
    CMS_REQUIRE(o.stream >= 0 && o.stream < n_streams, "program: op on stream %d but only %d streams given", o.stream,
                n_streams);
    hipStream_t s = (hipStream_t)streams[o.stream];
    static int share_flags = -1;
    if (share_flags < 0) {
        const char* e = getenv("CMS_PROG_FLAG_SHARE");
        share_flags = e ? atoi(e) : 1;
    }
    const int shared_slot = (share_flags && o.kind == OP_SYNC && p->prev_flag_slot >= 0 && o.from >= 0 && o.from < n_streams &&
                             p->prev_sync_from == streams[o.from]) ? p->prev_flag_slot : -1;
    p->prev_flag_slot = -1;
    switch (o.kind) {
    case OP_CONV: {
        Timed* t = nullptr;
        const bool head = o.conv.y32 != nullptr;
        if (p->timing_every > 0 && (head || (p->conv_seen++ % p->timing_every) == 0)) {
            if (p->timed_used == p->timed.size()) {
                Timed nt;
                nt.used = false;
                nt.head = false;
                nt.flops = 0.0;
                if (hipEventCreate(&nt.e0) != hipSuccess || hipEventCreate(&nt.e1) != hipSuccess) {
                    set_error("program: hipEventCreate failed");
                    return CMS_ELAUNCH;
                }
                p->timed.push_back(nt);
            }
            t = &p->timed[p->timed_used++];
            t->flops = o.flops;
            t->used = true;
            t->head = head;
            (void)hipEventRecord(t->e0, s);
        }
        const int rc = o.f32 ? cms_conv_igemm_f32(&o.conv, s) : cms_conv_igemm(&o.conv, s);
        if (t) (void)hipEventRecord(t->e1, s);
        p->last_head = (t && head) ? (long)(t - &p->timed[0]) : -1;
        p->last_head_stream = o.stream;
        return rc;
    }
    case OP_ASPP_GATHER: {
        const AsppOp& g = o.aspp;
        const int rc = cms_aspp_gather_fwd(g.src, g.bias, (float*)g.dst, g.tap_dy, g.tap_dx, g.n_taps, g.n, g.c, g.zc, g.h,
                                           g.w, s);
        if (p->last_head >= 0 && p->last_head_stream == o.stream) (void)hipEventRecord(p->timed[p->last_head].e1, s);
        p->last_head = -1;
        return rc;
    }
    case OP_ASPP_SPREAD: {
        const AsppOp& g = o.aspp;
        return cms_aspp_spread_bwd(g.src, g.dst, g.d_dtype, g.tap_dy, g.tap_dx, g.n_taps, g.n, g.c, g.zc, g.h, g.w, s);
    }
    case OP_WGRAD:
        return o.f32 ? cms_conv_wgrad_f32(&o.wg, s) : cms_conv_wgrad(&o.wg, s);
    case OP_WGRAD_GROUP:
        return cms_conv_wgrad_group_run(o.ptr, (int)o.bytes, o.from, o.f32, s);
    case OP_CHANNEL_SUM:
        return cms_channel_sum(o.ptr, o.f32, o.bytes, o.from, (float*)o.aspp.dst, s);
    case OP_WGRAD_FINISH:
        return cms_wgrad_finish_run(o.ptr, (int)o.bytes, o.from, s);
    case OP_BN: return cms_bn_run(&o.bn, s);
    case OP_MEMSET:
        if (hipMemsetAsync(o.ptr, 0, o.bytes, s) != hipSuccess) {
            set_error("program: hipMemsetAsync failed");
            return CMS_ELAUNCH;
        }
        return CMS_OK;
    case OP_SYNC: {
        CMS_REQUIRE(o.from >= 0 && o.from < n_streams, "program: sync from stream %d but only %d streams given", o.from,
                    n_streams);
        if (streams[o.from] == streams[o.stream]) return CMS_OK;
        if (p->use_flags && o.flag_slot < p->n_flags - 1) {
            int slot = shared_slot;
            unsigned val = p->prev_flag_val;
            if (slot < 0) {
                slot = o.flag_slot;
                val = ++p->seq;
                hipLaunchKernelGGL(sync_set_kernel, dim3(1), dim3(64), 0, (hipStream_t)streams[o.from], p->flags + slot, (int)val);
            }
            hipLaunchKernelGGL(sync_wait_kernel, dim3(1), dim3(64), 0, s, (const int*)(p->flags + slot), (int)val,
                               p->flags + (p->n_flags - 1));
            p->prev_flag_slot = slot;
            p->prev_flag_val = val;
            p->prev_sync_from = streams[o.from];
            return launch_status("program: flag sync");
        }
        if (hipEventRecord(o.ev, (hipStream_t)streams[o.from]) != hipSuccess ||
            hipStreamWaitEvent(s, o.ev, 0) != hipSuccess) {
            set_error("program: event record / wait failed");
            return CMS_ELAUNCH;
        }
        return CMS_OK;
    }
    }
    set_error("program: unknown op kind %d", o.kind);
    return CMS_EINVAL;
}

extern "C" int cms_program_create(cms_program** out) {
    CMS_REQUIRE(out != nullptr, "program_create: NULL out pointer");
    *out = new (std::nothrow) cms_program();
    CMS_REQUIRE(*out != nullptr, "program_create: out of host memory");
    return CMS_OK;
}
// ... 64 lines not shown
    o.kind = OP_WGRAD_FINISH; o.stream = stream_idx; o.group = group;
    o.ptr = const_cast<void*>(items_dev); o.bytes = (size_t)n_items; o.from = total_blocks;
    return push(p, o);
}

extern "C" int cms_program_add_memset(cms_program* p, void* ptr, size_t bytes, int stream_idx, int group) {
    CMS_REQUIRE(p && ptr && bytes > 0, "program_add_memset: NULL pointer / empty range");
    CMS_REQUIRE(stream_idx >= 0 && stream_idx < CMS_PROGRAM_MAX_STREAMS, "program_add_memset: stream index %d", stream_idx);
    Op o = {};
    o.kind = OP_MEMSET; o.stream = stream_idx; o.group = group; o.ptr = ptr; o.bytes = bytes;
    return push(p, o);
}

extern "C" int cms_program_add_sync(cms_program* p, int from_stream, int to_stream, int group) {
    CMS_REQUIRE(p, "program_add_sync: NULL program");
    CMS_REQUIRE(from_stream >= 0 && from_stream < CMS_PROGRAM_MAX_STREAMS && to_stream >= 0 &&
                    to_stream < CMS_PROGRAM_MAX_STREAMS, "program_add_sync: stream indices %d -> %d", from_stream, to_stream);
    Op o = {};
    o.kind = OP_SYNC; o.stream = to_stream; o.from = from_stream; o.group = group;
    o.flag_slot = p->n_syncs++;
    if (hipEventCreateWithFlags(&o.ev, hipEventDisableTiming) != hipSuccess) {
        set_error("program_add_sync: hipEventCreate failed");
        return CMS_ELAUNCH;
    }
    return push(p, o);
}

static int add_aspp(cms_program* p, int kind, const float* src, const float* bias, void* dst, int d_dtype, const int* dy,
                    const int* dx, int n_taps, int n, int c, int zc, int h, int w, int stream_idx, int group) {
    CMS_REQUIRE(p && src && dst && dy && dx, "program_add_aspp: NULL pointer");
    CMS_REQUIRE(n_taps > 0 && n_taps <= CMS_CONV_MAX_TAPS, "program_add_aspp: 1..%d taps", CMS_CONV_MAX_TAPS);
    CMS_REQUIRE(stream_idx >= 0 && stream_idx < CMS_PROGRAM_MAX_STREAMS, "program_add_aspp: stream index %d", stream_idx);
    Op o = {};
    o.kind = kind; o.stream = stream_idx; o.group = group;
    o.aspp.src = src; o.aspp.bias = bias; o.aspp.dst = dst; o.aspp.d_dtype = d_dtype;
    for (int i = 0; i < n_taps; ++i) { o.aspp.tap_dy[i] = dy[i]; o.aspp.tap_dx[i] = dx[i]; }
    o.aspp.n_taps = n_taps; o.aspp.n = n; o.aspp.c = c; o.aspp.zc = zc; o.aspp.h = h; o.aspp.w = w;
    return push(p, o);
}

extern "C" int cms_program_add_aspp_gather(cms_program* p, const float* z, const float* bias, float* logits, const int* tap_dy,
                                           const int* tap_dx, int n_taps, int n, int c, int zc, int h, int w, int stream_idx,
                                           int group) {
    return add_aspp(p, OP_ASPP_GATHER, z, bias, logits, CMS_F32, tap_dy, tap_dx, n_taps, n, c, zc, h, w, stream_idx, group);
}

extern "C" int cms_program_add_aspp_spread(cms_program* p, const float* dlogits, void* d_nhwc, int d_dtype, const int* tap_dy,
                                           const int* tap_dx, int n_taps, int n, int c, int zc, int h, int w, int stream_idx,
                                           int group) {
    return add_aspp(p, OP_ASPP_SPREAD, dlogits, nullptr, d_nhwc, d_dtype, tap_dy, tap_dx, n_taps, n, c, zc, h, w, stream_idx,
                    group);
}

extern "C" int cms_program_add_bn(cms_program* p, const cms_bn_op* op, int stream_idx, int group) {
    CMS_REQUIRE(p && op, "program_add_bn: NULL pointer");
    CMS_REQUIRE(op->what >= CMS_BN_REDUCE && op->what <= CMS_BN_BWD_SUMS_TILES, "program_add_bn: unknown op %d", op->what);
    CMS_REQUIRE((op->what != CMS_BN_FINALIZE_TILES && op->what != CMS_BN_BWD_SUMS_TILES) || (op->ws && op->tile_rows > 0),
                "program_add_bn: finalize_tiles / sums_tiles need the tile sums (ws) and the tile rows");
    CMS_REQUIRE(op->what != CMS_BN_BWD_SUMS_TILES || op->sums, "program_add_bn: sums_tiles writes `sums`");
    CMS_REQUIRE(op->groups <= 1 || op->ws || (op->what != CMS_BN_REDUCE && op->what != CMS_BN_REDUCE_BWD),
                "program_add_bn: grouped reductions need a workspace");
    CMS_REQUIRE(op->what != CMS_BN_REDUCE_BWD || !op->mask_bits || op->ws,
                "program_add_bn: the backward reduction reads mask bits on the workspace kernels only");
    CMS_REQUIRE(stream_idx >= 0 && stream_idx < CMS_PROGRAM_MAX_STREAMS, "program_add_bn: stream index %d", stream_idx);
    Op o = {};
    o.kind = OP_BN; o.stream = stream_idx; o.group = group;
    o.bn = *op;
    return push(p, o);
}

extern "C" int cms_program_size(const cms_program* p) { return p ? (int)p->ops.size() : 0; }

extern "C" int cms_program_sync_count(const cms_program* p) { return p ? p->n_syncs : 0; }

extern "C" int cms_program_set_sync_flags(cms_program* p, int* flags_dev, int n_flags) {
    CMS_REQUIRE(p, "program_set_sync_flags: NULL program");
    CMS_REQUIRE((flags_dev == nullptr && n_flags == 0) || (flags_dev != nullptr && n_flags >= 2),
                "program_set_sync_flags: a device buffer of >= 2 zeroed ints (one per sync op + the timeout counter), or NULL / 0");
    p->flags = flags_dev;
    p->n_flags = n_flags;
    return CMS_OK;
}

static void begin_replay(cms_program* p, void* const* streams) {
    static int flag_sync = -1;
    if (flag_sync < 0) {
        const char* e = getenv("CMS_PROG_FLAG_SYNC");
        flag_sync = e ? atoi(e) : 1;
    }
    p->prev_flag_slot = -1;
    p->use_flags = false;
    if (flag_sync != 0 && p->flags != nullptr && p->n_syncs > 0) {
        hipStreamCaptureStatus st = hipStreamCaptureStatusNone;
        if (hipStreamIsCapturing((hipStream_t)streams[0], &st) != hipSuccess) {
            (void)hipGetLastError();
            st = hipStreamCaptureStatusNone;
        }
        p->use_flags = st == hipStreamCaptureStatusNone;
    }
}

extern "C" int cms_program_run(cms_program* p, int first, int last, void* const* streams, int n_streams) {
    CMS_REQUIRE(p && streams && n_streams > 0, "program_run: NULL program / streams");
    const int n = (int)p->ops.size();
    if (last < 0 || last > n) last = n;
    CMS_REQUIRE(first >= 0 && first <= last, "program_run: bad range [%d, %d) of %d ops", first, last, n);
// ... 71 lines not shown
```

cutmix-semisup-seg_amd/ops.py:

```python
import ctypes as C

import numpy as np
import torch

from . import _lib
from ._lib import fn, check


def _stream():
    return C.c_void_p(torch.cuda.current_stream().cuda_stream)


def _ptr(t):
    return None if t is None else C.c_void_p(t.data_ptr())


def _need_cuda(*tensors):
    for t in tensors:
        if t is not None and not t.is_cuda:
            raise RuntimeError('cutmix-semisup-seg_amd ops run on the GPU only (got a {} tensor); there is no CPU '
                               'fallback'.format(t.device))


def _f32c(t):
# ... 59 lines not shown
    def __init__(self, loss_fn, conf_thresh, conf_per_pixel, align_corners):
        if loss_fn not in _lib.LOSS_IDS:
            raise ValueError('Unknown consistency loss function {}'.format(loss_fn))
        self.loss_fn = loss_fn
        self.conf_thresh = float(conf_thresh)
        self.conf_per_pixel = bool(conf_per_pixel)
        self.align_corners = bool(align_corners)

    def fill(self, d):
        d.align_corners = int(self.align_corners)
        d.loss_fn = _lib.LOSS_IDS[self.loss_fn]
        d.conf_thresh = self.conf_thresh
        d.conf_per_pixel = int(self.conf_per_pixel)


class ConsistencyConfig(_LossConfig):

    def __init__(self, mode='mix', loss_fn='var', conf_thresh=0.97, conf_per_pixel=False, align_corners=True,
                 invert=True):
        if mode not in ('mix', 'cut'):
            raise ValueError('Unknown mask_mode {}'.format(mode))
        _LossConfig.__init__(self, loss_fn, conf_thresh, conf_per_pixel, align_corners)
        self.mode = mode
        self.invert = bool(invert)


def _nonempty_ranges(ranges):
    if ranges is not None and ranges.dim() == 3 and ranges.shape[1] == 0:
        return torch.zeros((int(ranges.shape[0]), 1, 4), dtype=torch.int32, device=ranges.device)
    return ranges


def _cons_desc(cfg, l_stu, l_tea0, l_tea1, ranges, mask, um0, um1, out_size):
    n, c, h, w = (int(s) for s in l_stu.shape)
    d = _lib.ConsistencyDesc()
    d.l_stu, d.l_tea0, d.l_tea1 = l_stu.data_ptr(), l_tea0.data_ptr(), (l_tea1.data_ptr() if l_tea1 is not None else None)
    d.ranges = ranges.data_ptr() if ranges is not None else None
    d.mask = mask.data_ptr() if mask is not None else None
    d.um0 = um0.data_ptr() if um0 is not None else None
    d.um1 = um1.data_ptr() if um1 is not None else None
    d.n, d.c, d.h, d.w = n, c, h, w
    d.H, d.W = int(out_size[0]), int(out_size[1])
    cfg.fill(d)
    d.n_boxes = int(ranges.shape[1]) if ranges is not None else 0
    d.invert = int(cfg.invert)
    d.mode = _lib.MODE_MIX if cfg.mode == 'mix' else _lib.MODE_CUT
    return d


def _workspace(name, d, device):
    return torch.empty(max(int(fn['cms_{}_workspace_bytes'.format(name)](C.byref(d))), 16), dtype=torch.uint8, device=device)


def _check_grad_out(who, grad_out, like):
    if grad_out.dtype != torch.float32 or tuple(grad_out.shape) != tuple(like.shape) or not grad_out.is_contiguous():
        raise ValueError('{}: grad_out must be a contiguous f32 tensor of the logits\' shape'.format(who))


def _finalized_scalars(stats, stats_g, cfg, ramp_val, cons_weight):
    scalars = torch.empty(4, dtype=torch.float32, device=stats.device)
    check(fn['cms_consistency_finalize'](_ptr(stats), _ptr(stats_g), cfg.conf_thresh, int(cfg.conf_per_pixel),
                                         float(ramp_val), float(cons_weight), _ptr(scalars), _stream()),
          'cms_consistency_finalize')
    return scalars


def _allreduce_sum(t, group):
    import torch.distributed as dist
    if dist.is_available() and dist.is_initialized() and dist.get_world_size(group) > 1:
        dist.all_reduce(t, op=dist.ReduceOp.SUM, group=group)
        return True
    return False


def _cons_prepare(who, cfg, l_stu, l_tea0, l_tea1, out_size, ranges, mask, um0, um1, grad_out=None):
    _need_cuda(l_stu, l_tea0, l_tea1, ranges, mask, um0, um1, grad_out)
    l_stu, l_tea0, l_tea1 = _f32c(l_stu), _f32c(l_tea0), _f32c(l_tea1)
    mask, um0, um1 = _f32c(mask), _f32c(um0), _f32c(um1)
    ranges = _nonempty_ranges(ranges)
    if l_tea0.shape != l_stu.shape or (l_tea1 is not None and l_tea1.shape != l_stu.shape):
        raise ValueError('consistency: student / teacher logits shapes differ')
    if grad_out is not None:
        _check_grad_out(who, grad_out, l_stu)
    d = _cons_desc(cfg, l_stu, l_tea0, l_tea1, ranges, mask, um0, um1, out_size)
    return d, (l_stu, l_tea0, l_tea1, ranges, mask, um0, um1, cfg, tuple(int(v) for v in out_size))


def _cons_scalars(stats, cfg, ramp_val, cons_weight, group, sync_conf_rate):
    stats_g = stats
    if sync_conf_rate and cfg.conf_thresh > 0.0:
        g = stats.clone()
        if _allreduce_sum(g, group):
            stats_g = g
    return _finalized_scalars(stats, stats_g, cfg, ramp_val, cons_weight)


def consistency_forward(cfg, l_stu, l_tea0, l_tea1, out_size, ranges=None, mask=None, um0=None, um1=None,
                        ramp_val=1.0, cons_weight=1.0, group=None, sync_conf_rate=True):
    d, keep = _cons_prepare('consistency_forward', cfg, l_stu, l_tea0, l_tea1, out_size, ranges, mask, um0, um1)
    dev = keep[0].device
    ws = _workspace('consistency', d, dev)
    stats = torch.empty(4, dtype=torch.float64, device=dev)
    check(fn['cms_consistency_fwd'](C.byref(d), _ptr(ws), _ptr(stats), _stream()), 'cms_consistency_fwd')
    return _cons_scalars(stats, cfg, ramp_val, cons_weight, group, sync_conf_rate), (d, keep, stats)


def consistency_backward(ctx, scalars, grad_out=None, samples=None):
    d, keep, _ = ctx
    l_stu = keep[0]
    if grad_out is None:
        grad_out = torch.zeros_like(l_stu)
    if samples is not None:
        s0, s1 = int(samples[0]), int(samples[1])
        if not (0 <= s0 < s1 <= int(l_stu.shape[0])):
            raise ValueError('consistency_backward: bad sample range')
        sl = lambda t: None if t is None else t[s0:s1]
        l_s, l_t0, l_t1, ranges, mask, um0, um1, cfg, out_size = keep
        d = _cons_desc(cfg, sl(l_s), sl(l_t0), sl(l_t1), sl(ranges), sl(mask), sl(um0), sl(um1), out_size)
        check(fn['cms_consistency_bwd'](C.byref(d), _ptr(scalars), _ptr(grad_out[s0:s1]), _stream()), 'cms_consistency_bwd')
        return grad_out
    check(fn['cms_consistency_bwd'](C.byref(d), _ptr(scalars), _ptr(grad_out), _stream()), 'cms_consistency_bwd')
    return grad_out


def consistency_fused(cfg, l_stu, l_tea0, l_tea1, out_size, grad_out, ranges=None, mask=None, um0=None, um1=None,
                      ramp_val=1.0, cons_weight=1.0, group=None, sync_conf_rate=True):
    d, keep = _cons_prepare('consistency_fused', cfg, l_stu, l_tea0, l_tea1, out_size, ranges, mask, um0, um1, grad_out)
    l_stu, l_tea0, l_tea1, ranges, mask, um0, um1 = keep[:7]
    if not fn['cms_consistency_fused_supported'](C.byref(d)):
        sc, cctx = consistency_forward(cfg, l_stu, l_tea0, l_tea1, out_size, ranges, mask, um0, um1, ramp_val, cons_weight, group,
                                       sync_conf_rate)
        consistency_backward(cctx, sc, grad_out)
        return sc
    dev = l_stu.device
    ws = _workspace('consistency', d, dev)
    stats = torch.empty(4, dtype=torch.float64, device=dev)
    P = float(d.n) * float(d.H) * float(d.W)
    grad_unit = float(ramp_val) * float(cons_weight) / P
    check(fn['cms_consistency_fwd_bwd'](C.byref(d), grad_unit, _ptr(ws), _ptr(stats), _ptr(grad_out), _stream()),
          'cms_consistency_fwd_bwd')
    scalars = _cons_scalars(stats, cfg, ramp_val, cons_weight, group, sync_conf_rate)
    if cfg.conf_thresh > 0.0 and not cfg.conf_per_pixel:
        check(fn['cms_scale_by_scalar'](_ptr(grad_out), grad_out.numel(), _ptr(scalars), 1, 1.0, _stream()), 'cms_scale_by_scalar')
    return scalars


class _ConsistencyFn(torch.autograd.Function):
    @staticmethod
    def forward(ctx, l_stu, l_tea0, l_tea1, ranges, mask, um0, um1, cfg, out_size, ramp_val, cons_weight, group):
        scalars, c = consistency_forward(cfg, l_stu.detach(), l_tea0, l_tea1, out_size, ranges, mask, um0, um1,
                                         ramp_val, cons_weight, group)
        ctx.c = c
        ctx.scalars = scalars
        ctx.in_dtype = l_stu.dtype
        closs, rate, unsup = scalars[0], scalars[1], scalars[3]
        ctx.mark_non_differentiable(closs, rate)
        return unsup, closs, rate

    @staticmethod
    def backward(ctx, g_unsup, g_closs, g_rate):
        sc = ctx.scalars.clone()
        sc[2] = sc[2] * g_unsup
        grad = consistency_backward(ctx.c, sc)
        return (grad.to(ctx.in_dtype),) + (None,) * 11


def consistency_loss(l_stu, l_tea0, l_tea1, out_size, cfg, ranges=None, mask=None, um0=None, um1=None, ramp_val=1.0,
                     cons_weight=1.0, group=None):
    return _ConsistencyFn.apply(l_stu, l_tea0, l_tea1, ranges, mask, um0, um1, cfg, tuple(out_size), ramp_val,
                                cons_weight, group)


def _lam_vector(lam, n):
    lam = _f32c(lam).reshape(-1)
    if int(lam.numel()) != int(n):
        raise ValueError('ict: {} mix factors for {} samples'.format(int(lam.numel()), int(n)))
    return lam


def ict_blend(x0, x1, lam, out=None):
    _need_cuda(x0, x1, lam, out)
    if x0.shape != x1.shape or x0.dtype != x1.dtype:
        raise ValueError('ict_blend: x0/x1 shape or dtype mismatch')
    x0, x1 = x0.contiguous(), x1.contiguous()
    n = int(x0.shape[0])
    lam = _lam_vector(lam, n)
    if out is None:
        out = torch.empty_like(x0)
    elif out.shape != x0.shape or out.dtype != x0.dtype or not out.is_contiguous():
        raise ValueError('ict_blend: out must be a contiguous tensor of the inputs\' shape and dtype')
    if x0.numel() == 0:
        return out
    check(fn['cms_ict_blend'](_ptr(x0), _ptr(x1), _ptr(out), _dtype_code(x0), _ptr(lam), n, int(x0.numel()) // n, _stream()),
          'cms_ict_blend')
    return out

# ... 112 lines not shown
    d = _lib.CeDesc()
    d.logits, d.labels = logits.data_ptr(), labels.data_ptr()
    if labels.dtype == torch.uint8:
        d.label_dtype = _lib.LABEL_U8
    elif labels.dtype == torch.int64:
        d.label_dtype = _lib.LABEL_I64
    else:
        raise TypeError('labels must be uint8 or int64, got {}'.format(labels.dtype))
    d.ignore_index = int(ignore_index)
    d.n, d.c, d.h, d.w = n, c, h, w
    d.H, d.W = int(out_size[0]), int(out_size[1])
    d.align_corners = int(bool(align_corners))
    return d


def _ce_prepare(logits, labels, out_size, ignore_index, align_corners, grad_out=None):
    _need_cuda(logits, labels, grad_out)
    logits = _f32c(logits)
    labels = labels.contiguous()
    if labels.dim() == 4:
        labels = labels[:, 0].contiguous()
    if out_size is None:
        out_size = labels.shape[1:3]
    if tuple(labels.shape) != (logits.shape[0], int(out_size[0]), int(out_size[1])):
        raise ValueError('ce: labels shape {} does not match (N,H,W)=({}, {}, {})'.format(
            tuple(labels.shape), logits.shape[0], out_size[0], out_size[1]))
    if grad_out is not None:
        _check_grad_out('ce_fused', grad_out, logits)
    return _ce_desc(logits, labels, ignore_index, out_size, align_corners), logits, labels


def _ce_scalars(stats, loss_weight, group, sync_count):
    if sync_count:
        import torch.distributed as dist
        cnt = stats[1:2].clone()
        if _allreduce_sum(cnt, group):
            stats = torch.stack([stats[0], cnt[0] / dist.get_world_size(group)])
    scalars = torch.empty(2, dtype=torch.float32, device=stats.device)
    check(fn['cms_ce_finalize'](_ptr(stats), float(loss_weight), _ptr(scalars), _stream()), 'cms_ce_finalize')
    return scalars, stats


def ce_forward(logits, labels, out_size=None, ignore_index=255, align_corners=True, loss_weight=1.0, group=None,
               sync_count=False):
    d, logits, labels = _ce_prepare(logits, labels, out_size, ignore_index, align_corners)
    ws = _workspace('ce', d, logits.device)
    stats = torch.empty(2, dtype=torch.float64, device=logits.device)
    check(fn['cms_ce_fwd'](C.byref(d), _ptr(ws), _ptr(stats), _stream()), 'cms_ce_fwd')
    scalars, stats = _ce_scalars(stats, loss_weight, group, sync_count)
    return scalars, (d, (logits, labels), stats)


def ce_fused(logits, labels, grad_out, out_size=None, ignore_index=255, align_corners=True, loss_weight=1.0, group=None,
             sync_count=False):
    d, logits, labels = _ce_prepare(logits, labels, out_size, ignore_index, align_corners, grad_out)
    if not fn['cms_ce_fused_supported'](C.byref(d)):
        sc, cctx = ce_forward(logits, labels, out_size, ignore_index, align_corners, loss_weight, group, sync_count)
        ce_backward(cctx, sc, grad_out)
        return sc
    ws = _workspace('ce', d, logits.device)
    stats = torch.empty(2, dtype=torch.float64, device=logits.device)
    check(fn['cms_ce_fwd_bwd'](C.byref(d), _ptr(ws), _ptr(stats), _ptr(grad_out), _stream()), 'cms_ce_fwd_bwd')
    scalars, _ = _ce_scalars(stats, loss_weight, group, sync_count)
    check(fn['cms_scale_by_scalar'](_ptr(grad_out), grad_out.numel(), _ptr(scalars), 1, 1.0, _stream()), 'cms_scale_by_scalar')
    return scalars


def ce_backward(ctx, scalars, grad_out=None):
    d, keep, _ = ctx
    if grad_out is None:
        grad_out = torch.zeros_like(keep[0])
    check(fn['cms_ce_bwd'](C.byref(d), _ptr(scalars), _ptr(grad_out), _stream()), 'cms_ce_bwd')
    return grad_out


class _CeFn(torch.autograd.Function):
    @staticmethod
    def forward(ctx, logits, labels, out_size, ignore_index, align_corners):
        scalars, c = ce_forward(logits.detach(), labels, out_size, ignore_index, align_corners)
        ctx.c = c
        ctx.scalars = scalars
        ctx.in_dtype = logits.dtype
        return scalars[0]

    @staticmethod
    def backward(ctx, g):
        sc = ctx.scalars.clone()
        sc[1] = sc[1] * g
        return ce_backward(ctx.c, sc).to(ctx.in_dtype), None, None, None, None


def cross_entropy(logits, labels, out_size=None, ignore_index=255, align_corners=True):
    return _CeFn.apply(logits, labels, None if out_size is None else tuple(out_size), ignore_index, align_corners)


class _UpsampleFn(torch.autograd.Function):
    @staticmethod
    def forward(ctx, x, size, align_corners):
        _need_cuda(x)
        xin = _f32c(x)
        n, c, h, w = (int(s) for s in xin.shape)
        H, W = int(size[0]), int(size[1])
        out = torch.empty((n, c, H, W), dtype=torch.float32, device=x.device)
        check(fn['cms_upsample_bilinear_fwd'](_ptr(xin), _ptr(out), n, c, h, w, H, W, int(bool(align_corners)),
                                              _stream()), 'cms_upsample_bilinear_fwd')
        ctx.geo = (n, c, h, w, H, W, int(bool(align_corners)))
        ctx.in_dtype = x.dtype
        return out

    @staticmethod
    def backward(ctx, g):
        n, c, h, w, H, W, ac = ctx.geo
        g = _f32c(g)
        gi = torch.empty((n, c, h, w), dtype=torch.float32, device=g.device)
        check(fn['cms_upsample_bilinear_bwd'](_ptr(g), _ptr(gi), n, c, h, w, H, W, ac, _stream()),
              'cms_upsample_bilinear_bwd')
        return gi.to(ctx.in_dtype), None, None
# ... 861 lines not shown
    n, _, h, w = (int(v) for v in x_shape)
    dx = torch.empty((n, 3, h, w), dtype=torch.float32, device=ds.device)
    check(fn['cms_stem_dgrad'](_ptr(ds), _dtype_code(ds), _ptr(w147), _ptr(scale), _ptr(dx), n, h, w, _stream()),
          'cms_stem_dgrad')
    return dx


def bn_fold(flat, idx_weight, idx_bias, idx_mean, idx_var, eps, scale, bias):
    _need_cuda(flat, idx_weight, idx_bias, idx_mean, idx_var, scale, bias)
    n = int(scale.numel())
    if flat.dtype != torch.float32 or scale.dtype != torch.float32 or bias.dtype != torch.float32 \
            or any(t.dtype != torch.int64 or int(t.numel()) != n or not t.is_contiguous() for t in (idx_weight, idx_bias, idx_mean, idx_var)) \
            or int(bias.numel()) != n or not (scale.is_contiguous() and bias.is_contiguous() and flat.is_contiguous()):
        raise TypeError('bn_fold: fp32 arena / outputs and int64 index tables of the outputs\' length required')
    check(fn['cms_bn_fold'](_ptr(flat), _ptr(idx_weight), _ptr(idx_bias), _ptr(idx_mean), _ptr(idx_var), n, float(eps), _ptr(scale),
                            _ptr(bias), _stream()), 'cms_bn_fold')


HBM_PEAK_BPS, MFMA_PEAK_FLOPS = 8.0e12, 2.5e15


class Program(object):

    def __init__(self):
        h = C.c_void_p()
        check(fn['cms_program_create'](C.byref(h)), 'cms_program_create')
        self.h = h
        self.keep = []
        self.marks = []
        self.group = 0
        self.flops = 0.0
        self.conv_launches = 0
        self.conv_bytes = 0.0
        self.head_bytes = 0.0
        self.head_bytes_alg = 0.0
        self.floor_s = 0.0
        self.head_launches = 0
        self.by_route = {}
        self.n_streams = 1
        self.bn_kinds = {}
        self.host_ops = []

    def __del__(self):
        h, self.h = getattr(self, 'h', None), None
        if h is not None:
            try:
                fn['cms_program_destroy'](h)
            except Exception:
                pass

    def size(self):
        return int(fn['cms_program_size'](self.h))

    def mark(self, tag):
        self.marks.append((self.size(), tag))

    @staticmethod
    def _handles(streams):
        arr = (C.c_void_p * len(streams))()
        for i, st in enumerate(streams):
            arr[i] = st.cuda_stream
        return arr

    def _ensure_sync_flags(self, force=False):
        if not force and _os.environ.get('CMS_PROG_FLAG_SYNC', '0') != '1':
            return
        n = int(fn['cms_program_sync_count'](self.h))
        if n > 0 and getattr(self, '_sync_flags_n', 0) != n:
            if getattr(self, 'sync_flags', None) is not None:
                self.keep.append(self.sync_flags)
            self.sync_flags = torch.zeros(n + 1, dtype=torch.int32, device=torch.device('cuda', torch.cuda.current_device()))
            self._sync_flags_n = n
            check(fn['cms_program_set_sync_flags'](self.h, self.sync_flags.data_ptr(), n + 1), 'cms_program_set_sync_flags')

    def sync_timeouts(self):
        fl = getattr(self, 'sync_flags', None)
        return 0 if fl is None else int(fl[-1].item())

    def run(self, streams, first=0, last=-1):
        if len(streams) < self.n_streams:
            raise ValueError('program recorded on {} streams, {} given'.format(self.n_streams, len(streams)))
        self._ensure_sync_flags()
        if self.host_ops:
            size = self.size()
            end = size if (last < 0 or last >= size) else int(last)
            handles = self._handles(streams)
            pos = int(first)
            for idx, si, call in self.host_ops:
                if idx < pos or idx > end or (idx == end and end != size):
                    continue
                if idx > pos:
                    check(fn['cms_program_run'](self.h, pos, idx, handles, len(streams)), 'cms_program_run')
                    pos = idx
                with torch.cuda.stream(streams[si]):
                    call()
            if pos < end:
                check(fn['cms_program_run'](self.h, pos, end, handles, len(streams)), 'cms_program_run')
            return
        check(fn['cms_program_run'](self.h, int(first), int(last), self._handles(streams), len(streams)),
              'cms_program_run')

    def set_timing(self, every_k):
        check(fn['cms_program_set_timing'](self.h, int(every_k)), 'cms_program_set_timing')

    def read_timing(self):
        ms, fl, n = C.c_double(), C.c_double(), C.c_long()
# ... 53 lines not shown
    if _REC is None:
        t.zero_()
        return t
    if not t.is_contiguous():
        raise TypeError('memset_zero: contiguous tensor required')
    prog = _REC[0]
    idx = fn['cms_program_add_memset'](prog.h, _ptr(t), t.numel() * t.element_size(), _rec_stream_index(), prog.group)
    if idx < 0:
        check(idx, 'cms_program_add_memset')
    prog.keep.append(t)
    return t


def stream_wait(waiter, waited):
    if _REC is None:
        waiter.wait_stream(waited)
        return
    prog = _REC[0]
    idx = fn['cms_program_add_sync'](prog.h, _rec_stream_index(waited), _rec_stream_index(waiter), prog.group)
    if idx < 0:
        check(idx, 'cms_program_add_sync')


def _tap_arrays(taps):
    n = len(taps)
    dy = (C.c_int * n)(*[int(t[0]) for t in taps])
    dx = (C.c_int * n)(*[int(t[1]) for t in taps])
    return dy, dx, n


def aspp_gather_fwd(z, bias, taps, num_classes, out=None):
    _need_cuda(z, bias, out)
    if z.dtype != torch.float32 or not z.is_contiguous():
        raise TypeError('aspp_gather_fwd: contiguous fp32 (N, ZC, h, w) input required')
    n, zc, h, w = (int(v) for v in z.shape)
    if out is None:
        out = torch.empty((n, int(num_classes), h, w), dtype=torch.float32, device=z.device)
    dy, dx, nt = _tap_arrays(taps)
    if _REC is not None:
        prog = _REC[0]
        idx = fn['cms_program_add_aspp_gather'](prog.h, _ptr(z), _ptr(bias), _ptr(out), dy, dx, nt, n, int(num_classes), zc,
                                                h, w, _rec_stream_index(), prog.group)
        if idx < 0:
            check(idx, 'cms_program_add_aspp_gather')
        prog.keep += [t for t in (z, bias, out) if t is not None]
        prog.head_bytes += 4.0 * nt * int(num_classes) * n * h * w + 4.0 * out.numel()
        prog.head_bytes_alg += 4.0 * out.numel()
        return out
    check(fn['cms_aspp_gather_fwd'](_ptr(z), _ptr(bias), _ptr(out), dy, dx, nt, n, int(num_classes), zc, h, w, _stream()),
          'cms_aspp_gather_fwd')
    return out


def aspp_spread_bwd(dlogits, taps, zc, dtype, out=None):
    _need_cuda(dlogits, out)
    if dlogits.dtype != torch.float32 or not dlogits.is_contiguous():
        raise TypeError('aspp_spread_bwd: contiguous fp32 (N, C, h, w) gradient required')
    n, c, h, w = (int(v) for v in dlogits.shape)
    if out is None:
        out = torch.empty((n, h, w, int(zc)), dtype=dtype, device=dlogits.device)
    dy, dx, nt = _tap_arrays(taps)
    if _REC is not None:
        prog = _REC[0]
        idx = fn['cms_program_add_aspp_spread'](prog.h, _ptr(dlogits), _ptr(out), _dtype_code(out), dy, dx, nt, n, c,
                                                int(zc), h, w, _rec_stream_index(), prog.group)
        if idx < 0:
            check(idx, 'cms_program_add_aspp_spread')
        prog.keep += [dlogits, out]
        return out
    check(fn['cms_aspp_spread_bwd'](_ptr(dlogits), _ptr(out), _dtype_code(out), dy, dx, nt, n, c, int(zc), h, w, _stream()),
          'cms_aspp_spread_bwd')
    return out


_ZERO_PAGES = {}


def _zero_page(device):
    z = _ZERO_PAGES.get(device)
    if z is None:
        z = torch.zeros(32768, dtype=torch.bfloat16, device=device)
        _ZERO_PAGES[device] = z
    return z


_CONV8_WS = {}
_ROUTE_NAMES = {8: 'conv8_kernel', 2: 'conv_igemm_mixed_kernel', 1: 'conv_igemm_kernel<2, 2, 2, 2', 3: 'conv_igemm_kernel<1, 4, 2, 1',
                4: 'conv_igemm_kernel<1, 4, 1, 1', 0: 'other'}


def conv8_workspace(device):
    if _REC is not None:
        prog = _REC[0]
        store, key = prog.__dict__.setdefault('conv8_ws', {}), _rec_stream_index()
    else:
        store, key = _CONV8_WS, (device.index, int(torch.cuda.current_stream().cuda_stream))
    ws = store.get(key)
    if ws is None:
        n = int(fn['cms_conv_igemm_workspace_bytes']())
        ws = torch.empty(n, dtype=torch.uint8, device=device)
        ws[:65536].zero_()
        store[key] = ws
    return ws


def conv_taps(kh, kw, dilation, padding):
    return [(ky * dilation - padding, kx * dilation - padding) for ky in range(kh) for kx in range(kw)]


def conv_igemm(x, w_packed, taps, stride=1, out_hw=None, scale=None, bias=None, res=None, relu=False, mode=0,
               mask_src=None, out=None, out_f32_nchw=None, cout_real=None, out_stride=1, out_full_hw=None, tile=0,
               ksplit=1, variant=0, out_pixel_offset=0, mask_bits_out=None, mask_bits=None, stats=None,
               mask_gates_res=False):
    _need_cuda(x, w_packed, scale, bias, res, mask_src, out, out_f32_nchw, mask_bits_out, mask_bits)
    for t in (mask_bits_out, mask_bits):
        if t is not None and (t.dtype != torch.uint8 or not t.is_contiguous() or x.dtype != torch.bfloat16):
            raise TypeError('conv_igemm: ReLU mask bits are contiguous uint8 tensors of the bf16 entry point')
    if mask_bits is not None and mask_src is not None:
        raise ValueError('conv_igemm: mask_bits replaces mask_src')
    if mask_gates_res and (mask_bits is None or res is None or int(mode) != 1):
        raise ValueError('conv_igemm: mask_gates_res needs a data-gradient launch with res and mask_bits')
    if x.dtype not in (torch.bfloat16, torch.float32) or w_packed.dtype != x.dtype or not x.is_contiguous() \
            or not w_packed.is_contiguous():
        raise TypeError('conv_igemm: contiguous NHWC input and packed weights of one dtype (bf16 or fp32) required')
# ... 381 lines not shown
```

cutmix-semisup-seg_amd/step.py:

```python
import os
import torch

from . import ops
from .graph_replay import GraphReplay


class StepConfig(object):
    def __init__(self, mask_mode='mix', cons_loss_fn='var', cons_weight=1.0, conf_thresh=0.97, conf_per_pixel=False,
                 rampup=-1, unsup_batch_ratio=1, invert=True, fuse_batches=True, compute_dtype=torch.bfloat16,
                 overlap_teacher=True, bucketed_allreduce=True, allreduce_dtype='fp32', deterministic=False,
                 early_optimizer=False):
        if mask_mode not in ('mix', 'zero', 'cut'):
            raise ValueError('Unknown mask_mode {}'.format(mask_mode))
        self.mix = mask_mode == 'mix'
        self.cons_weight = float(cons_weight)
        self.rampup = rampup
        self.unsup_batch_ratio = int(unsup_batch_ratio)
        self.fuse_batches = bool(fuse_batches)
        self.overlap_teacher = bool(overlap_teacher)
        self.bucketed_allreduce = bool(bucketed_allreduce)
        if allreduce_dtype not in ('fp32', 'bf16'):
            raise ValueError('allreduce_dtype must be fp32 or bf16')
        self.allreduce_dtype = allreduce_dtype
        self.deterministic = bool(deterministic)
# ... 310 lines not shown

    def _separate_or_graphed(self, sup_x, sup_y, unsup_batches, ramp, out_size, use_unsup):
        cfg = self.cfg
        if not (sup_x.is_cuda and self._graph_wanted() and (cfg.rampup <= 0 or float(ramp) >= 1.0)):
            return self._separate_passes(sup_x, sup_y, unsup_batches, ramp, out_size, use_unsup)
        flat = [sup_x, sup_y]
        for u in (unsup_batches if use_unsup else ()):
            flat += [u.x0_tea, u.x1_tea, u.x0_stu, u.x1_stu, u.ranges, u.um0, u.um1, u.mask]
        extra = (float(ramp), tuple(out_size), bool(use_unsup), self.student.training, self.teacher.training,
                 getattr(self.student, 'compute_dtype', None), getattr(self.teacher, 'compute_dtype', None))

        def passes(ts, capturing):
            ubs = [UnsupBatch(x0t, rg, um0=m0, x1_tea=x1t, um1=m1, x0_stu=x0s, x1_stu=x1s, mask=mk)
                   for x0t, x1t, x0s, x1s, rg, m0, m1, mk in (ts[i:i + 8] for i in range(2, len(ts), 8))]
            overlap = not capturing or os.environ.get('CMS_STEP_GRAPH_OVERLAP', '1') != '0'
            return self._separate_passes(ts[0], ts[1], ubs, ramp, out_size, use_unsup, allow_overlap=overlap)

        return self._graphs.run(flat, extra, passes, nets=(self.student, self.teacher), device=sup_x.device)

    def _fused_passes(self, sup_x, sup_y, unsup_batches, ramp, out_size, use_unsup, independent, groups):
        cfg = self.cfg
        n_sup = sup_x.shape[0]
        stu_in = [sup_x]
        tea_in = []
        zev = None
        if use_unsup:
            main = torch.cuda.current_stream()
            side = self._teacher_stream() if (cfg.overlap_teacher and self.teacher is not self.student) else main
            if side is not main:
                side.wait_stream(main)
            zev = self._zero_grad(main)
            for ub in unsup_batches:
                tea_in.append(ub.x0_tea)
                if cfg.mix:
                    tea_in.append(ub.x1_tea)
            with torch.cuda.stream(side):
                x_tea = torch.cat(tea_in, dim=0) if len(tea_in) > 1 else tea_in[0]
            for ub in unsup_batches:
                stu_in.append(self._student_inputs(ub))
        else:
            self.student_optim.zero_grad()
        x_stu = torch.cat(stu_in, dim=0) if len(stu_in) > 1 else stu_in[0]
        if use_unsup and side is not main and self._both_on_executor():
            from .backbone_hip import run_body_pair
            with torch.cuda.stream(side), torch.no_grad():
                xt = self.teacher.stem_nhwc(x_tea)
            xs = self.student.stem_nhwc(x_stu)
            stu_lo, tea_lo = run_body_pair(self.student.hip_executor(), xs, self.teacher.hip_executor(), xt, side)
        else:
            if use_unsup:
                with torch.cuda.stream(side), torch.no_grad():
                    tea_lo = self.teacher.forward_lowres(x_tea)
            stu_lo = self.student.forward_lowres(x_stu)
        grad_lo = torch.zeros(stu_lo.shape, dtype=torch.float32, device=stu_lo.device)
        lo_det = stu_lo.detach()
        split = use_unsup and side is not main
        if split:
            side.wait_stream(main)
        cons_vals = []

        def consistency_branch():
            s_off, t_off = n_sup, 0
            for ub in unsup_batches:
                n = ub.x0_tea.shape[0]
                l0 = tea_lo[t_off:t_off + n]
                l1 = tea_lo[t_off + n:t_off + 2 * n] if cfg.mix else None
                t_off += 2 * n if cfg.mix else n
                sc = ops.consistency_fused(cfg.cons, lo_det[s_off:s_off + n], l0, l1, out_size, grad_lo[s_off:s_off + n],
                                           ranges=ub.ranges, mask=ub.mask, um0=ub.um0, um1=ub.um1, ramp_val=ramp,
                                           cons_weight=cfg.cons_weight, group=self.group)
                s_off += n
                if split and isinstance(sc, torch.Tensor):
                    sc.record_stream(main)
                cons_vals.append(sc)
        if split:
            with torch.cuda.stream(side):
                consistency_branch()
        ce_sc = ops.ce_fused(lo_det[:n_sup], sup_y, grad_lo[:n_sup], out_size, 255, self.align_corners, group=self.group)
        sex = self._student_executor()
        if split:
            if independent and groups is None and sex is not None and hasattr(sex, '_refresh_for_backward'):
                sex._refresh_for_backward()
            main.wait_stream(side)
        elif use_unsup:
            consistency_branch()
        ex = self._arm_buckets() or self._arm_early_optimizer()
        dex = sex if sex is not None and hasattr(sex, 'join_wgrad') else None
        if dex is not None:
            dex.defer_wgrad_join = True
        if zev is not None:
            main.wait_event(zev)
        try:
            stu_lo.backward(grad_lo.to(stu_lo.dtype))
        finally:
            if ex is not None:
                ex.grad_hook = None
            if dex is not None:
                dex.defer_wgrad_join = False
                dex.join_wgrad()
        return ce_sc, cons_vals

    def __call__(self, sup_x, sup_y, unsup_batches, ramp_val=1.0):
        cfg = self.cfg
        out_size = sup_x.shape[2:4]
        use_unsup = cfg.cons_weight > 0.0 and len(unsup_batches) > 0
        ramp = ramp_val if cfg.rampup > 0 else 1.0

        independent = self._samples_independent()
        groups = None if (independent or not cfg.fuse_batches) else self._sample_groups(sup_x.shape[0], unsup_batches, use_unsup)
        if groups is not None:
            self.student.set_sample_groups(groups[0])
            if use_unsup:
                self.teacher.set_sample_groups(groups[1])
        try:
            if cfg.fuse_batches and (independent or groups is not None):
                ce_sc, cons_vals = self._fused_passes(sup_x, sup_y, unsup_batches, ramp, out_size, use_unsup, independent, groups)
            else:
                ce_sc, cons_vals = self._separate_or_graphed(sup_x, sup_y, unsup_batches, ramp, out_size, use_unsup)

            ops.join_side_streams()
            self._allreduce_grads()
            if self._early_armed:
                self._early_armed = False
                torch.cuda.current_stream().wait_stream(self._opt_stream)
            self.student_optim.step()
            if self.teacher_optim is not None:
                self.teacher_optim.step()
            self._post_nan_probe(ce_sc[0])
            return step_result(ce_sc, cons_vals)
        finally:
            if groups is not None:
                self.student.set_sample_groups(1)
                self.teacher.set_sample_groups(1)
```

include/cutmixseg.h:

```cpp
#ifndef CUTMIXSEG_H
#define CUTMIXSEG_H

#include <stddef.h>
#include <stdint.h>

#ifdef __cplusplus
extern "C" {
#endif

#define CMS_VERSION 101

#define CMS_OK 0
#define CMS_EINVAL (-1)
#define CMS_ELAUNCH (-2)
#define CMS_EUNSUPPORTED (-3)

#define CMS_F32 0
#define CMS_BF16 1

#define CMS_LABEL_U8 0
#define CMS_LABEL_I64 1

#define CMS_LOSS_VAR 0
#define CMS_LOSS_LOGITS_VAR 1
#define CMS_LOSS_LOGITS_SMOOTHL1 2
#define CMS_LOSS_BCE 3
#define CMS_LOSS_KLD 4

#define CMS_MODE_MIX 0
#define CMS_MODE_CUT 1

int cms_version(void);
const char* cms_last_error(void);
int cms_device_info(int* n_cu, char* name_out, size_t name_cap);


int cms_boxmask_rasterize(const int32_t* ranges, int n, int n_boxes, int h, int w, int invert,
                          float* mask_out, void* stream);

int cms_cutmix_paste(const void* x0, const void* x1, void* out, int dtype, const int32_t* ranges, int n,
                     int n_boxes, int c, int h, int w, int invert, void* stream);

int cms_cutmix_paste_mask(const void* x0, const void* x1, void* out, int dtype, const float* mask, int n, int c,
                          int h, int w, void* stream);

typedef struct cms_consistency_desc {
    const float* l_stu;
    const float* l_tea0;
    const float* l_tea1;
    const int32_t* ranges;
    const float* mask;
    const float* um0;
    const float* um1;
    int n, c, h, w;
    int H, W;
    int align_corners;
    int n_boxes, invert;
    int mode;
    int loss_fn;
    float conf_thresh;
    int conf_per_pixel;
} cms_consistency_desc;

size_t cms_consistency_workspace_bytes(const cms_consistency_desc* d);

int cms_consistency_fwd(const cms_consistency_desc* d, void* workspace, double* stats_out, void* stream);

int cms_consistency_finalize(const double* stats_local, const double* stats_global, float conf_thresh,
                             int conf_per_pixel, float ramp_val, float cons_weight, float* scalars_out,
                             void* stream);

int cms_consistency_bwd(const cms_consistency_desc* d, const float* scalars, float* grad_l_stu, void* stream);

int cms_consistency_fused_supported(const cms_consistency_desc* d);
int cms_consistency_fwd_bwd(const cms_consistency_desc* d, float grad_unit, void* workspace, double* stats_out,
                            float* grad_l_stu, void* stream);
int cms_scale_by_scalar(float* x, long long n, const float* scalars, int index, float factor, void* stream);

typedef struct cms_ce_desc {
    const float* logits;
    const void* labels;
    int label_dtype;
    int ignore_index;
    int n, c, h, w, H, W, align_corners;
} cms_ce_desc;

size_t cms_ce_workspace_bytes(const cms_ce_desc* d);
int cms_ce_fwd(const cms_ce_desc* d, void* workspace, double* stats_out, void* stream);
int cms_ce_finalize(const double* stats, float loss_weight, float* scalars_out, void* stream);
int cms_ce_bwd(const cms_ce_desc* d, const float* scalars, float* grad_logits, void* stream);
int cms_ce_fused_supported(const cms_ce_desc* d);
int cms_ce_fwd_bwd(const cms_ce_desc* d, void* workspace, double* stats_out, float* grad_logits, void* stream);
int cms_loss_set_deterministic(int on);


int cms_ict_blend(const void* x0, const void* x1, void* out, int dtype, const float* lam, int n, long long chw, void* stream);

typedef struct cms_ict_desc {
    const float* l_stu;
    const float* l_tea0;
    const float* l_tea1;
    const float* lam;
    const float* um0;
    const float* um1;
    int n, c, h, w;
    int H, W;
    int align_corners;
    int loss_fn;
    float conf_thresh;
    int conf_per_pixel;
} cms_ict_desc;

size_t cms_ict_workspace_bytes(const cms_ict_desc* d);

int cms_ict_fwd(const cms_ict_desc* d, void* workspace, double* stats_out, void* stream);

int cms_ict_bwd(const cms_ict_desc* d, const void* workspace, const float* scalars, float* grad_l_stu, void* stream);


typedef struct cms_aug_desc {
    const float* l_stu;
    const float* l_tea;
    const float* xf;
    const float* um0;
    const float* um1;
    int n, c, h, w;
    int H, W;
    int align_corners;
    int loss_fn;
    float conf_thresh;
    int conf_per_pixel;
    int force_global;
} cms_aug_desc;

size_t cms_aug_workspace_bytes(const cms_aug_desc* d);

int cms_aug_fwd(const cms_aug_desc* d, void* workspace, double* stats_out, void* stream);

int cms_aug_bwd(const cms_aug_desc* d, const float* scalars, float* grad_l_stu, void* stream);

int cms_upsample_bilinear_fwd(const float* lo, float* hi, int n, int c, int h, int w, int H, int W,
                              int align_corners, void* stream);
int cms_upsample_bilinear_bwd(const float* grad_hi, float* grad_lo, int n, int c, int h, int w, int H, int W,
                              int align_corners, void* stream);

// ... 190 lines not shown
int cms_stage_batch(const cms_stage_desc* d, void* stream);
int cms_stage_luma(const cms_stage_desc* d, float* luma, void* stream);

enum cms_bn_what { CMS_BN_REDUCE = 0, CMS_BN_FINALIZE, CMS_BN_APPLY, CMS_BN_REDUCE_BWD, CMS_BN_BWD_APPLY, CMS_BN_COUNT,
                   CMS_BN_STATS, CMS_BN_FINALIZE_TILES, CMS_BN_BWD_SUMS_TILES };

typedef struct cms_bn_op {
    int what;
    int dtype, c, relu;
    const void* x;
    const void* res;
    void* y;
    const void* dy;
    void* dx;
    void* dres;
    double* sums;
    const float* gamma;
    const float* beta;
    float* mean;
    float* rstd;
    float* scale;
    float* shift;
    float* running_mean;
    float* running_var;
    long long* counter;
    double* clear_a;
    double* clear_b;
    void* ws;
    double count;
    unsigned long long n_pixels;
    float eps, momentum;
    int groups;
    int tile_rows;
    void* mask_bits;
} cms_bn_op;

size_t cms_bn_workspace_bytes(size_t n_pixels, int c, int groups);
int cms_bn_run(const cms_bn_op* op, void* stream);
int cms_frozen_bn_act_bwd(const void* dy, const void* y, void* dx, void* dres, int dtype, const float* scale, size_t n_pixels, int c,
                          void* stream);

int cms_channel_copy(const void* src, size_t src_pitch, void* dst, size_t dst_pitch, size_t rows, int channels, int dtype,
                     size_t row_div, void* stream);
int cms_add_n(const void* const* srcs, int k, void* dst, size_t n, int dtype, void* stream);
int cms_rows_reduce(const void* src, size_t pitch, int n, size_t rows_per_sample, int channels, int dtype, float* dst,
                    float scale, void* stream);
int cms_upsample_nhwc(const void* src, void* dst, size_t dst_pitch, int n, int h, int w, int H, int W, int channels, int dtype,
                      int align_corners, int backward, void* stream);

int cms_aspp_gather_fwd(const float* z, const float* bias, float* logits, const int* tap_dy, const int* tap_dx, int n_taps,
                        int n, int c, int zc, int h, int w, void* stream);
int cms_aspp_spread_bwd(const float* dlogits, void* d_nhwc, int d_dtype, const int* tap_dy, const int* tap_dx, int n_taps,
                        int n, int c, int zc, int h, int w, void* stream);

int cms_stem_pack_weights(const void* w_khkwcoci, int w_dtype, float* w_packed, void* stream);
int cms_stem_out_hw(int h, int w, int* ho, int* wo, int* hp, int* wp);
int cms_stem_fwd(const void* x_nchw, int x_dtype, void* y_nhwc, int y_dtype, const float* w_packed, const float* scale,
                 const float* bias, int n, int h, int w, void* stream);
int cms_maxpool3x3s2_fwd(const void* s_nhwc, void* p_nhwc, uint8_t* argmax, int dtype, int n, int hs, int ws, int c,
                         int ceil_mode, void* stream);
int cms_maxpool3x3s2_relu_bwd(const void* dp_nhwc, const uint8_t* argmax, const void* s_nhwc, void* ds_nhwc, int dtype,
                              int n, int hs, int ws, int c, int ceil_mode, void* stream);
int cms_stem_wgrad(const void* x_nchw, int x_dtype, const void* ds_nhwc, int ds_dtype, float* dw_khkwcoci,
                   const float* scale, int n, int h, int w, void* stream);
long long cms_stem_wgrad_workspace_bytes(int x_dtype, int ds_dtype, int n, int h, int w);
int cms_stem_wgrad_ws(const void* x_nchw, int x_dtype, const void* ds_nhwc, int ds_dtype, float* dw_khkwcoci,
                      const float* scale, int n, int h, int w, void* workspace, long long workspace_bytes, void* stream);
int cms_stem_dgrad(const void* ds_nhwc, int ds_dtype, const float* w_packed, const float* scale, float* dx_nchw, int n,
                   int h, int w, void* stream);

#define CMS_PROGRAM_MAX_STREAMS 4
typedef struct cms_program cms_program;
int cms_program_create(cms_program** out);
int cms_program_destroy(cms_program* p);
int cms_program_add_conv(cms_program* p, const cms_conv_desc* d, int f32, int stream_idx, int group);
int cms_program_add_wgrad(cms_program* p, const cms_wgrad_desc* d, int f32, int stream_idx, int group);
int cms_program_add_wgrad_group(cms_program* p, const void* table_dev, int n_items, int total_blocks, int kind, int stream_idx,
                                int group);
int cms_program_add_memset(cms_program* p, void* ptr, size_t bytes, int stream_idx, int group);
int cms_program_add_aspp_gather(cms_program* p, const float* z, const float* bias, float* logits, const int* tap_dy,
                                const int* tap_dx, int n_taps, int n, int c, int zc, int h, int w, int stream_idx, int group);
int cms_program_add_aspp_spread(cms_program* p, const float* dlogits, void* d_nhwc, int d_dtype, const int* tap_dy,
                                const int* tap_dx, int n_taps, int n, int c, int zc, int h, int w, int stream_idx, int group);
int cms_program_add_sync(cms_program* p, int from_stream, int to_stream, int group);
int cms_program_sync_count(const cms_program* p);
int cms_program_set_sync_flags(cms_program* p, int* flags_dev, int n_flags);
typedef struct cms_wfinish_item {
    float* scratch;
    float* grad;
    const uint16_t* w;
    const float* scale;
    float* wdot;
    int ntaps, cout, cin;
    int first_block;
} cms_wfinish_item;
int cms_channel_sum(const void* src, int dtype, size_t rows, int channels, float* dst, void* stream);
int cms_wgrad_finish_pack(cms_wfinish_item* items, int n_items);
int cms_wgrad_finish_run(const void* items_dev, int n_items, int total_blocks, void* stream);
int cms_program_add_channel_sum(cms_program* p, const void* src, int dtype, size_t rows, int channels, float* dst, int stream_idx,
                                int group);
int cms_program_add_wgrad_finish(cms_program* p, const void* items_dev, int n_items, int total_blocks, int stream_idx, int group);

int cms_program_add_bn(cms_program* p, const cms_bn_op* op, int stream_idx, int group);
int cms_program_size(const cms_program* p);
int cms_program_run(cms_program* p, int first, int last, void* const* streams, int n_streams);
int cms_program_run_pair(cms_program* a, void* const* streams_a, int na, cms_program* b, void* const* streams_b, int nb);
int cms_program_set_timing(cms_program* p, int every_k);
int cms_program_read_timing(cms_program* p, double* sum_ms, double* sum_flops, long* launches, double* head_ms,
                            long* head_launches);

int cms_fft2(void* data, int batch, int fh, int fw, int inverse, const void* tw_h, const void* tw_w, void* stream);

typedef struct cms_pd_patch {
    long long img_off;
    int hs, ws;
    int cy, cx;
} cms_pd_patch;
int cms_pd_load_image(const uint8_t* pool_img, const cms_stage_entry* entry_host, int ph, int pw, int fh, int fw, void* planes,
                      int64_t* sq, void* stream);
int cms_pd_load_patches(const uint8_t* pool_img, const cms_pd_patch* patches, int n, int ph, int pw, int fh, int fw, void* planes,
                        void* stream);
int cms_pd_patch_sqdiff(const uint8_t* pool_img, const cms_pd_patch* a, const cms_pd_patch* b, int n, int ph, int pw, int64_t* out,
                        void* stream);
int cms_pd_spectrum_product(const void* f_img, const void* f_pairs, int n_pairs, int fh, int fw, void* out, void* stream);
int cms_pd_finish(const void* corr, const int64_t* p2, const int64_t* q2, int n, int h, int w, int fh, int fw, int64_t* d2,
                  int64_t* keys, uint64_t* residual_bits, void* stream);
size_t cms_select_workspace_bytes(int n);
int cms_select_k_smallest(const int64_t* keys, const uint8_t* mask, const uint8_t* labels, const int32_t* cls, int mode, int n,
                          long long m, int k, int64_t* out, int32_t* count, void* workspace, size_t workspace_bytes, void* stream);

int cms_pd_box_sum(const void* in, int in_is_int64, int hp, int wp, int ph, int pw, void* work, int64_t* out, void* stream);
size_t cms_pd_neighbour_workspace_bytes(int hs, int ws, int ph, int pw);
int cms_pd_neighbour_maps(const uint8_t* pool_img, const cms_stage_entry* entry_host, int ph, int pw, void* work, int64_t* out_d2,
                          void* stream);

int cms_downsample_image_u8(const uint8_t* src, int n, int h, int w, int d, uint8_t* dst, void* stream);
// ... 11 lines not shown
```

Baseline: 643.1 images/sec.

## Fold loss finalize and gradient scaling into loss kernels via per-row scale

```diff
diff --git a/cutmix-semisup-seg_amd/_lib.py b/cutmix-semisup-seg_amd/_lib.py
--- a/cutmix-semisup-seg_amd/_lib.py
+++ b/cutmix-semisup-seg_amd/_lib.py
@@ -154,6 +154,10 @@
     'cms_consistency_fused_supported': (c_int, [_P(ConsistencyDesc)]),
     'cms_consistency_fwd_bwd': (c_int, [_P(ConsistencyDesc), c_float, c_void_p, c_void_p, c_void_p, c_void_p]),
     'cms_scale_by_scalar': (c_int, [c_void_p, C.c_longlong, c_void_p, c_int, c_float, c_void_p]),
+    'cms_consistency_fwd_bwd_finish': (c_int, [_P(ConsistencyDesc), c_float, c_float, c_float, c_void_p, c_void_p, c_void_p, c_void_p,
+                                               c_void_p, c_void_p]),
+    'cms_loss_workspace_head_bytes': (c_size_t, []),
+    'cms_loss_workspace_status': (c_int, [c_void_p, c_void_p]),
     'cms_ict_blend': (c_int, [c_void_p, c_void_p, c_void_p, c_int, c_void_p, c_int, C.c_longlong, c_void_p]),
     'cms_ict_workspace_bytes': (c_size_t, [_P(IctDesc)]),
     'cms_ict_fwd': (c_int, [_P(IctDesc), c_void_p, c_void_p, c_void_p]),
@@ -167,6 +171,7 @@
     'cms_ce_bwd': (c_int, [_P(CeDesc), c_void_p, c_void_p, c_void_p]),
     'cms_ce_fused_supported': (c_int, [_P(CeDesc)]),
     'cms_ce_fwd_bwd': (c_int, [_P(CeDesc), c_void_p, c_void_p, c_void_p, c_void_p]),
+    'cms_ce_fwd_bwd_finish': (c_int, [_P(CeDesc), c_float, c_void_p, c_void_p, c_void_p, c_void_p, c_void_p, c_void_p]),
     'cms_upsample_bilinear_fwd': (c_int, [c_void_p, c_void_p, c_int, c_int, c_int, c_int, c_int, c_int, c_int,
                                           c_void_p]),
     'cms_upsample_bilinear_bwd': (c_int, [c_void_p, c_void_p, c_int, c_int, c_int, c_int, c_int, c_int, c_int,
@@ -220,6 +225,8 @@
                                     c_int, c_void_p]),
     'cms_aspp_spread_bwd': (c_int, [c_void_p, c_void_p, c_int, _P(c_int), _P(c_int), c_int, c_int, c_int, c_int, c_int,
                                     c_int, c_void_p]),
+    'cms_aspp_spread_bwd_scaled': (c_int, [c_void_p, c_void_p, c_void_p, c_int, _P(c_int), _P(c_int), c_int, c_int, c_int, c_int,
+                                           c_int, c_int, c_void_p]),
     'cms_stem_pack_weights': (c_int, [c_void_p, c_int, c_void_p, c_void_p]),
     'cms_stem_out_hw': (c_int, [c_int, c_int, _P(c_int), _P(c_int), _P(c_int), _P(c_int)]),
     'cms_stem_fwd': (c_int, [c_void_p, c_int, c_void_p, c_int, c_void_p, c_void_p, c_void_p, c_int, c_int, c_int,
@@ -245,6 +252,8 @@
                                             c_int, c_int, c_int, c_int, c_int, c_int]),
     'cms_program_add_aspp_spread': (c_int, [c_void_p, c_void_p, c_void_p, c_int, _P(c_int), _P(c_int), c_int, c_int, c_int,
                                             c_int, c_int, c_int, c_int, c_int]),
+    'cms_program_add_aspp_spread_scaled': (c_int, [c_void_p, c_void_p, c_void_p, c_void_p, c_int, _P(c_int), _P(c_int), c_int, c_int,
+                                                   c_int, c_int, c_int, c_int, c_int, c_int]),
     'cms_program_add_bn': (c_int, [c_void_p, _P(BnOp), c_int, c_int]),
     'cms_program_size': (c_int, [c_void_p]),
     'cms_program_run': (c_int, [c_void_p, c_int, c_int, _P(c_void_p), c_int]),
diff --git a/cutmix-semisup-seg_amd/backbone_hip.py b/cutmix-semisup-seg_amd/backbone_hip.py
--- a/cutmix-semisup-seg_amd/backbone_hip.py
+++ b/cutmix-semisup-seg_amd/backbone_hip.py
@@ -89,6 +89,8 @@
         self.wgrad_streams = 2 if os.environ.get('CMS_WGRAD8', '1') != '0' else 1
         self.defer_wgrad_join = False
         self._pending_join = None
+        self._dl_bufs = {}
+        self.pending_row_scale = None
         self._sides = []
         self.conv_tile = 0
         self.tile_rules = {}
@@ -388,10 +390,10 @@
     def _wgrad_raw(self, du, x, c):
         ops.conv_wgrad(du, x, c.taps, self.arena.packed(c.wkey, self.arena.grad), stride=c.stride, wg_target=self._wg_target())
 
-    def _backward_chain_bn(self, saved, dlg, want_w, sides, hook, box=None):
+    def _backward_chain_bn(self, saved, dlg, want_w, sides, hook, box=None, row_scale=None):
         x4 = saved[-1]
         main = torch.cuda.current_stream()
-        d = ops.aspp_spread_bwd(dlg, self.aspp_taps, self.aspp_zc, self.dtype)
+        d = ops.aspp_spread_bwd(dlg, self.aspp_taps, self.aspp_zc, self.dtype, row_scale=row_scale)
         dwall = None
         if want_w:
             dwall = torch.empty((1, self.aspp_zc, 2048), dtype=torch.float32, device=d.device)
@@ -628,12 +630,25 @@
             self._refresh_backward_weights()
             self._wT_version = self.version
 
-    def _head_bias_grads(self, dlogits, want_w, side=None):
+    def dlogit_buffers(self, shape, device):
+        key = tuple(int(v) for v in shape)
+        b = self._dl_bufs.get(key)
+        if b is None:
+            dev = torch.device(device)
+            b = self._dl_bufs[key] = [torch.empty(key, dtype=torch.float32, device=dev),
+                                      torch.ones(key[0], dtype=torch.float32, device=dev), True]
+        return b[0], b[1]
+
+    def _head_bias_grads(self, dlogits, want_w, side=None, row_scale=None):
         if want_w:
             if side is not None:
                 side.wait_stream(torch.cuda.current_stream())
                 dlogits.record_stream(side)
+                if row_scale is not None:
+                    row_scale.record_stream(side)
             with torch.cuda.stream(side if side is not None else torch.cuda.current_stream()):
+                if row_scale is not None:
+                    dlogits = dlogits * row_scale.view(-1, 1, 1, 1)
                 db = dlogits.sum(dim=(0, 2, 3))
                 for k in self.aspp_keys:
                     self.arena.view(k + '.bias', self.arena.grad).add_(db)
@@ -654,10 +669,10 @@
         l2, l3, l4 = self._layer_first[1], self._layer_first[2], self._layer_first[3]
         return sorted(set([0, l2, l3, (l3 + l4 + 1) // 2, l4]))
 
-    def _backward_chain(self, saved, dlg, want_w, sides, hook, box=None):
+    def _backward_chain(self, saved, dlg, want_w, sides, hook, box=None, row_scale=None):
         x4 = saved[-1]
         main = torch.cuda.current_stream()
-        d = ops.aspp_spread_bwd(dlg, self.aspp_taps, self.aspp_zc, self.dtype)
+        d = ops.aspp_spread_bwd(dlg, self.aspp_taps, self.aspp_zc, self.dtype, row_scale=row_scale)
         dwall = None
         keep = []
         if want_w:
@@ -710,13 +725,18 @@
         if want_w and self._grad_sentinel().grad is None:
             self.arena.ensure_grads_attached()
         n, _, h, w = dlogits.shape
+        row_scale, self.pending_row_scale = self.pending_row_scale, None
+        if row_scale is not None and int(row_scale.numel()) != int(n):
+            raise ValueError('pending_row_scale holds {} factors for a logit gradient of {} samples'.format(row_scale.numel(), n))
+        if row_scale is not None and tuple(int(v) for v in dlogits.shape) in self._dl_bufs:
+            self._dl_bufs[tuple(int(v) for v in dlogits.shape)][2] = False
         main = torch.cuda.current_stream()
         sides = self._side_streams(self.wgrad_streams) if (self.overlap_wgrad and want_w) else []
         hside = sides[0] if (sides and not bn) else None
         if not self.use_programs:
             if self.defer_wgrad_join and sides:
                 self._pending_join = list(sides)
-            self._head_bias_grads(dlogits, want_w, hside)
+            self._head_bias_grads(dlogits, want_w, hside, row_scale)
             box = {}
 
             def hook(bi):
@@ -725,7 +745,7 @@
                     box['done'] = True
                 if self.grad_hook is not None:
                     self.grad_hook(bi)
-            dx, dwall = chain(token, dlogits, want_w, sides, hook, box)
+            dx, dwall = chain(token, dlogits, want_w, sides, hook, box, row_scale=row_scale)
             if dwall is not None and 'done' not in box:
                 self._finish_head(dwall, hside)
             return dx
@@ -740,14 +760,24 @@
         prog = fprog.bwd.get(key)
         if prog is None:
             prog = ops.Program()
-            dlg = torch.empty(tuple(dlogits.shape), dtype=torch.float32, device=dlogits.device)
+            dlg, rs = self.dlogit_buffers(dlogits.shape, dlogits.device)
             streams = [main] + sides
             with ops.recording(prog, streams):
-                dx, dwall = chain(fprog.saved, dlg, want_w, sides, prog.mark)
-            prog.dlg, prog.dx, prog.dwall = dlg, dx, dwall
+                dx, dwall = chain(fprog.saved, dlg, want_w, sides, prog.mark, row_scale=rs)
+            prog.dlg_in, prog.row_scale, prog.dx, prog.dwall = dlg, rs, dx, dwall
             fprog.bwd[key] = prog
-        prog.dlg.copy_(dlogits)
-        self._head_bias_grads(dlogits, want_w, hside)
+        if dlogits.data_ptr() != prog.dlg_in.data_ptr():
+            prog.dlg_in.copy_(dlogits)
+        state = self._dl_bufs[tuple(int(v) for v in dlogits.shape)]
+        if row_scale is None:
+            if not state[2]:
+                prog.row_scale.fill_(1.0)
+                state[2] = True
+        else:
+            state[2] = False
+            if row_scale.data_ptr() != prog.row_scale.data_ptr():
+                prog.row_scale.copy_(row_scale)
+        self._head_bias_grads(dlogits, want_w, hside, row_scale)
         streams = [main] + sides
         if self.grad_hook is None or not want_w:
             prog.run(streams)
@@ -1333,6 +1363,7 @@
         ctx.executor = ex_stu
         ctx.saved_acts = saved
         ctx.mark_non_differentiable(logits_t)
+        ctx.set_materialize_grads(False)
         return logits_s, logits_t
 
     @staticmethod
diff --git a/cutmix-semisup-seg_amd/csrc/aspp.hip b/cutmix-semisup-seg_amd/csrc/aspp.hip
--- a/cutmix-semisup-seg_amd/csrc/aspp.hip
+++ b/cutmix-semisup-seg_amd/csrc/aspp.hip
@@ -43,8 +43,8 @@
 }
 
 template <class T>
-__global__ __launch_bounds__(256) void aspp_spread_bwd_kernel(const float* __restrict__ dl, T* __restrict__ d, AsppTaps tp,
-                                                              int N, int C, int ZC, int H, int W) {
+__global__ __launch_bounds__(256) void aspp_spread_bwd_kernel(const float* __restrict__ dl, const float* __restrict__ row_scale,
+                                                              T* __restrict__ d, AsppTaps tp, int N, int C, int ZC, int H, int W) {
     __shared__ short sdy[CMS_CONV_MAX_TAPS], sdx[CMS_CONV_MAX_TAPS];
     taps_to_lds(tp, sdy, sdx);
     const int n_taps = tp.n_taps;
@@ -59,6 +59,7 @@
         const int y = (int)(t % (unsigned)H);
         const int n = (int)(t / (unsigned)H);
         const float* dn = dl + (size_t)n * C * plane;
+        const float rs = row_scale ? row_scale[n] : 1.0f;
         float v[8];
         int k = (int)((ch * 8u) / (unsigned)C), c = (int)(ch * 8u) - k * C;
 #pragma unroll
@@ -68,6 +69,7 @@
                 const int yy = y - sdy[k], xx = x - sdx[k];
                 if ((unsigned)yy < (unsigned)H && (unsigned)xx < (unsigned)W) val = dn[(size_t)c * plane + (size_t)yy * W + xx];
             }
+            if (row_scale) val *= rs;
             v[e] = val;
             if (++c == C) { c = 0; ++k; }
         }
@@ -116,6 +118,11 @@
 
 extern "C" int cms_aspp_spread_bwd(const float* dlogits, void* d_nhwc, int d_dtype, const int* tap_dy, const int* tap_dx,
                                    int n_taps, int n, int c, int zc, int h, int w, void* stream) {
+    return cms_aspp_spread_bwd_scaled(dlogits, nullptr, d_nhwc, d_dtype, tap_dy, tap_dx, n_taps, n, c, zc, h, w, stream);
+}
+
+extern "C" int cms_aspp_spread_bwd_scaled(const float* dlogits, const float* row_scale, void* d_nhwc, int d_dtype, const int* tap_dy,
+                                          const int* tap_dx, int n_taps, int n, int c, int zc, int h, int w, void* stream) {
     CMS_REQUIRE(dlogits && d_nhwc, "aspp_spread_bwd: NULL pointer");
     CMS_REQUIRE(d_dtype == CMS_F32 || d_dtype == CMS_BF16, "aspp_spread_bwd: bad dtype");
     CMS_REQUIRE(n > 0 && c > 0 && h > 0 && w > 0 && zc >= n_taps * c, "aspp_spread_bwd: bad geometry (zc >= taps * classes)");
@@ -128,9 +135,9 @@
     hipStream_t s = (hipStream_t)stream;
     if (d_dtype == CMS_F32)
         hipLaunchKernelGGL(aspp_spread_bwd_kernel<float>, dim3(grid_for(total, 256, 256 * 16)), dim3(256), 0, s, dlogits,
-                           (float*)d_nhwc, tp, n, c, zc, h, w);
+                           row_scale, (float*)d_nhwc, tp, n, c, zc, h, w);
     else
         hipLaunchKernelGGL(aspp_spread_bwd_kernel<uint16_t>, dim3(grid_for(total, 256, 256 * 16)), dim3(256), 0, s, dlogits,
-                           (uint16_t*)d_nhwc, tp, n, c, zc, h, w);
+                           row_scale, (uint16_t*)d_nhwc, tp, n, c, zc, h, w);
     return launch_status("cms_aspp_spread_bwd");
 }
diff --git a/cutmix-semisup-seg_amd/csrc/loss_tiles.hpp b/cutmix-semisup-seg_amd/csrc/loss_tiles.hpp
--- a/cutmix-semisup-seg_amd/csrc/loss_tiles.hpp
+++ b/cutmix-semisup-seg_amd/csrc/loss_tiles.hpp
@@ -199,6 +199,95 @@
     if (threadIdx.x == 0) {
 #pragma unroll
         for (int k = 0; k < K; ++k) partials[blockIdx.x * K + k] = acc[k];
+    }
+}
+
+constexpr size_t LOSS_WS_HEAD = 16;
+struct LossFinish {
+    unsigned* head;
+    double* stats;
+    float* scalars;
+    float* row_scale;
+    int n_rows, nblocks, extra_slot;
+    double extra;
+};
+inline LossFinish no_finish() {
+    LossFinish f;
+    f.head = nullptr; f.stats = nullptr; f.scalars = nullptr; f.row_scale = nullptr;
+    f.n_rows = f.nblocks = 0; f.extra_slot = -1; f.extra = 0.0;
+    return f;
+}
+template <int K>
+constexpr size_t finish_lds_bytes() { return (size_t)K * 256 * sizeof(double); }
+
+template <class T>
+__device__ __forceinline__ T load_kernarg(size_t offset) {
+    static_assert(sizeof(T) % 4 == 0, "whole dwords");
+    typedef const __attribute__((address_space(4))) uint32_t* kptr;
+    kptr p = (kptr)((const __attribute__((address_space(4))) char*)__builtin_amdgcn_kernarg_segment_ptr() + offset);
+    uint32_t w[sizeof(T) / 4];
+#pragma unroll
+    for (size_t i = 0; i < sizeof(T) / 4; ++i) w[i] = p[i];
+    T v;
+    __builtin_memcpy(&v, w, sizeof(T));
+    return v;
+}
+
+template <int K>
+__device__ __noinline__ void sum_partials_ordered(const float* partials, int nblocks, double* sm) {
+    const int tid = threadIdx.x;
+    double loc[K];
+#pragma unroll
+    for (int k = 0; k < K; ++k) loc[k] = 0.0;
+    for (int i = tid; i < nblocks; i += 256) {
+#pragma unroll
+        for (int k = 0; k < K; ++k) loc[k] += (double)__hip_atomic_load(partials + i * K + k, __ATOMIC_RELAXED, __HIP_MEMORY_SCOPE_AGENT);
+    }
+#pragma unroll
+    for (int k = 0; k < K; ++k) sm[k * 256 + tid] = loc[k];
+    __syncthreads();
+    for (int s = 128; s > 0; s >>= 1) {
+        if (tid < s) {
+#pragma unroll
+            for (int k = 0; k < K; ++k) sm[k * 256 + tid] += sm[k * 256 + tid + s];
+        }
+        __syncthreads();
+    }
+}
+
+template <int K, class Finalize>
+__device__ __forceinline__ void store_partials_finish(float (&acc)[K], float* red, float* partials, const LossFinish& f, double* sm,
+                                                      Finalize finalize) {
+    if (f.head == nullptr) {
+        store_partials<K>(acc, red, partials);
+        return;
+    }
+    block_sum<K>(acc, red);
+    const int tid = threadIdx.x;
+    int* flag = reinterpret_cast<int*>(red) + 15;
+    if (tid == 0) {
+#pragma unroll
+        for (int k = 0; k < K; ++k) __hip_atomic_store(partials + blockIdx.x * K + k, acc[k], __ATOMIC_RELAXED, __HIP_MEMORY_SCOPE_AGENT);
+        asm volatile("s_waitcnt vmcnt(0)" ::: "memory");
+        const unsigned ticket = __hip_atomic_fetch_add(f.head, 1u, __ATOMIC_RELAXED, __HIP_MEMORY_SCOPE_AGENT);
+        if (ticket >= (unsigned)f.nblocks) __hip_atomic_store(f.head + 1, 1u, __ATOMIC_RELAXED, __HIP_MEMORY_SCOPE_AGENT);
+        *flag = ticket == (unsigned)(f.nblocks - 1);
+    }
+    __syncthreads();
+    if (*flag == 0) return;
+    sum_partials_ordered<K>(partials, f.nblocks, sm);
+    if (tid == 0) {
+        double sums[K + 1];
+#pragma unroll
+        for (int k = 0; k < K; ++k) sums[k] = sm[k * 256];
+        sums[K] = f.extra;
+#pragma unroll
+        for (int k = 0; k < K; ++k) f.stats[k] = sums[k];
+        if (f.extra_slot >= 0) f.stats[f.extra_slot] = f.extra;
+        const float rs = finalize(sums, f.scalars);
+        if (f.row_scale)
+            for (int i = 0; i < f.n_rows; ++i) f.row_scale[i] = rs;
+        __hip_atomic_store(f.head, 0u, __ATOMIC_RELAXED, __HIP_MEMORY_SCOPE_AGENT);
     }
 }
 
diff --git a/cutmix-semisup-seg_amd/csrc/losses.hip b/cutmix-semisup-seg_amd/csrc/losses.hip
--- a/cutmix-semisup-seg_amd/csrc/losses.hip
+++ b/cutmix-semisup-seg_amd/csrc/losses.hip
@@ -97,9 +97,8 @@
     store_partials<3>(acc, red, partials);
 }
 
-__global__ void cons_finalize_kernel(const double* __restrict__ sl, const double* __restrict__ sg, float tau,
-                                     int per_pixel, float ramp, float weight, float* __restrict__ out) {
-    if (threadIdx.x != 0 || blockIdx.x != 0) return;
+__device__ __forceinline__ void cons_finalize_values(const double* sl, const double* sg, float tau, int per_pixel, float ramp,
+                                                     float weight, float* __restrict__ out) {
     const double Pl = sl[3];
     double closs, gs, rate;
     if (tau > 0.0f) {
@@ -121,6 +120,12 @@
     out[1] = (float)rate;
     out[2] = (float)(gs * (double)ramp * (double)weight);
     out[3] = (float)(closs * (double)weight);
+}
+
+__global__ void cons_finalize_kernel(const double* __restrict__ sl, const double* __restrict__ sg, float tau,
+                                     int per_pixel, float ramp, float weight, float* __restrict__ out) {
+    if (threadIdx.x != 0 || blockIdx.x != 0) return;
+    cons_finalize_values(sl, sg, tau, per_pixel, ramp, weight, out);
 }
 
 template <int CT>
@@ -195,9 +200,16 @@
     tiled_scatter(g, stage, pixel_grad, grad, smem);
 }
 
+struct ConsTail {
+    LossFinish fin;
+    float ramp, weight;
+};
+struct ConsFusedParams {
+    ConsArgs a; float grad_unit; float* grad; int patch_stride; float* partials; ConsTail tail;
+};
 template <int CT, int LF>
 __global__ __launch_bounds__(256, (LF >= 0 && CT > 0) ? 4 : 1) void cons_fused_tiled_kernel(ConsArgs a, float grad_unit, float* __restrict__ grad,
-                                                               int patch_stride, float* __restrict__ partials) {
+                                                               int patch_stride, float* __restrict__ partials, ConsTail) {
     extern __shared__ __attribute__((aligned(16))) float smem[];
     const Geo& g = a.g;
     const bool pp = a.tau > 0.0f && a.d.conf_per_pixel;
@@ -232,7 +244,11 @@
     };
     tiled_scatter(g, stage, pixel_grad, grad, smem);
     __shared__ float red[3 * 16];
-    store_partials<3>(acc, red, partials);
+    const ConsTail t = load_kernarg<ConsTail>(offsetof(ConsFusedParams, tail));
+    store_partials_finish<3>(acc, red, partials, t.fin, reinterpret_cast<double*>(smem), [&](const double* sums, float* out) -> float {
+        cons_finalize_values(sums, sums, a.tau, a.d.conf_per_pixel, t.ramp, t.weight, out);
+        return (a.tau > 0.0f && !a.d.conf_per_pixel) ? out[1] : 1.0f;
+    });
 }
 
 __global__ __launch_bounds__(256) void scale_by_scalar_kernel(float* __restrict__ x, size_t n, const float* __restrict__ scalars,
@@ -307,10 +323,14 @@
     store_partials<2>(acc, red, partials);
 }
 
+__device__ __forceinline__ void ce_finalize_values(const double* stats, float weight, float* __restrict__ out) {
+    out[0] = (float)(stats[0] / stats[1]);
+    out[1] = stats[1] > 0.0 ? (float)((double)weight / stats[1]) : 0.0f;
+}
+
 __global__ void ce_finalize_kernel(const double* __restrict__ stats, float weight, float* __restrict__ out) {
     if (threadIdx.x != 0 || blockIdx.x != 0) return;
-    out[0] = (float)(stats[0] / stats[1]);
-    out[1] = stats[1] > 0.0 ? (float)((double)weight / stats[1]) : 0.0f;
+    ce_finalize_values(stats, weight, out);
 }
 
 template <int CT>
@@ -358,8 +378,15 @@
     tiled_scatter(g, stage, pixel_grad, grad, smem);
 }
 
+struct CeTail {
+    LossFinish fin;
+    float weight, pad;
+};
+struct CeFusedParams {
+    CeArgs a; float* grad; float* partials; CeTail tail;
+};
 template <int CT>
-__global__ __launch_bounds__(256) void ce_fused_tiled_kernel(CeArgs a, float* __restrict__ grad, float* __restrict__ partials) {
+__global__ __launch_bounds__(256) void ce_fused_tiled_kernel(CeArgs a, float* __restrict__ grad, float* __restrict__ partials, CeTail) {
     extern __shared__ __attribute__((aligned(16))) float smem[];
     const Geo& g = a.g;
     float acc[2] = {0.0f, 0.0f};
@@ -384,7 +411,11 @@
     };
     tiled_scatter(g, stage, pixel_grad, grad, smem);
     __shared__ float red[2 * 16];
-    store_partials<2>(acc, red, partials);
+    const CeTail t = load_kernarg<CeTail>(offsetof(CeFusedParams, tail));
+    store_partials_finish<2>(acc, red, partials, t.fin, reinterpret_cast<double*>(smem), [&](const double* sums, float* out) -> float {
+        ce_finalize_values(sums, t.weight, out);
+        return out[1];
+    });
 }
 
 static int g_loss_deterministic = -1;
@@ -459,31 +490,27 @@
     return a;
 }
 
-template <int K, class Kern, class... Args>
-static void launch_fused(Kern kern, int tiles, size_t lds, hipStream_t s, float* partials, double* stats_out, double extra, int extra_slot,
-                         Args... args) {
+template <int K, class Kern, class Tail, class... Args>
+static void launch_fused(Kern kern, int tiles, size_t lds, hipStream_t s, void* workspace, double* stats_out, double extra, int extra_slot,
+                         float* scalars_out, float* row_scale, int n_rows, Tail tail, Args... args) {
+    LossFinish f = no_finish();
+    float* partials = (float*)workspace;
+    if (scalars_out) {
+        f.head = (unsigned*)workspace;
+        partials = (float*)((char*)workspace + LOSS_WS_HEAD);
+        f.stats = stats_out; f.scalars = scalars_out; f.row_scale = row_scale;
+        f.n_rows = n_rows; f.nblocks = tiles; f.extra_slot = extra_slot; f.extra = extra;
+        lds = std::max(lds, finish_lds_bytes<K>());
+    }
+    tail.fin = f;
     allow_lds(kern, lds);
-    hipLaunchKernelGGL(kern, dim3(tiles), dim3(256), lds, s, args..., partials);
-    hipLaunchKernelGGL((reduce_partials_kernel<K>), dim3(1), dim3(256), 0, s, partials, tiles, stats_out, extra, extra_slot);
-}
-
-}
-
-using namespace cms;
-
-extern "C" size_t cms_consistency_workspace_bytes(const cms_consistency_desc* d) {
-    if (!d) return 0;
-    const Geo g = geo_of(d);
-    return (size_t)std::max(fwd_blocks(g, 3), fused_tiles(g, 3)) * 3 * sizeof(float);
-}
-
-extern "C" int cms_consistency_fused_supported(const cms_consistency_desc* d) {
-    if (check_cons(d)) return 0;
-    return fused_tiles(geo_of(d), 3) > 0 ? 1 : 0;
-}
-
-extern "C" int cms_consistency_fwd_bwd(const cms_consistency_desc* d, float grad_unit, void* workspace, double* stats_out,
-                                       float* grad_l_stu, void* stream) {
+    hipLaunchKernelGGL(kern, dim3(tiles), dim3(256), lds, s, args..., partials, tail);
+    if (!scalars_out)
+        hipLaunchKernelGGL((reduce_partials_kernel<K>), dim3(1), dim3(256), 0, s, partials, tiles, stats_out, extra, extra_slot);
+}
+
+static int cons_fwd_bwd(const cms_consistency_desc* d, float grad_unit, float ramp, float weight, void* workspace, double* stats_out,
+                        float* scalars_out, float* row_scale, float* grad_l_stu, void* stream) {
     int rc = check_cons(d);
     if (rc) return rc;
     CMS_REQUIRE(workspace && stats_out && grad_l_stu, "consistency_fwd_bwd: workspace / stats_out / grad NULL");
@@ -492,12 +519,73 @@
     CMS_REQUIRE(tiles > 0, "consistency_fwd_bwd: not available for this geometry / mode (ask cms_consistency_fused_supported)");
     hipStream_t s = (hipStream_t)stream;
     const int pstride = (int)patch_floats(d->c, a.g.sy, a.g.sx, TILE_H);
+    ConsTail tail;
+    tail.ramp = ramp; tail.weight = weight;
     CMS_DISPATCH_C(d->c, {
         auto kern = d->loss_fn == CMS_LOSS_VAR ? cons_fused_tiled_kernel<CT, LOSS_VAR> : cons_fused_tiled_kernel<CT, -1>;
-        launch_fused<3>(kern, tiles, tile_lds_bytes(d->c, a.g.sy, a.g.sx, 3), s, (float*)workspace, stats_out,
-                        (double)((size_t)d->n * d->H * d->W), 3, a, grad_unit, grad_l_stu, pstride);
+        launch_fused<3>(kern, tiles, tile_lds_bytes(d->c, a.g.sy, a.g.sx, 3), s, workspace, stats_out,
+                        (double)((size_t)d->n * d->H * d->W), 3, scalars_out, row_scale, d->n, tail, a, grad_unit, grad_l_stu, pstride);
     });
     return launch_status("cms_consistency_fwd_bwd");
+}
+
+static int ce_fwd_bwd(const cms_ce_desc* d, float weight, void* workspace, double* stats_out, float* scalars_out, float* row_scale,
+                      float* grad_logits, void* stream) {
+    int rc = check_ce(d);
+    if (rc) return rc;
+    CMS_REQUIRE(workspace && stats_out && grad_logits, "ce_fwd_bwd: workspace / stats_out / grad NULL");
+    const CeArgs a = make_ce_args(d);
+    const int tiles = fused_tiles(a.g, 1);
+    CMS_REQUIRE(tiles > 0, "ce_fwd_bwd: not available for this geometry / mode (ask cms_ce_fused_supported)");
+    CeTail tail;
+    tail.weight = weight; tail.pad = 0.0f;
+    CMS_DISPATCH_C(d->c, launch_fused<2>(ce_fused_tiled_kernel<CT>, tiles, tile_lds_bytes(d->c, a.g.sy, a.g.sx, 1), (hipStream_t)stream,
+                                         workspace, stats_out, 0.0, -1, scalars_out, row_scale, d->n, tail, a, grad_logits));
+    return launch_status("cms_ce_fwd_bwd");
+}
+
+}
+
+using namespace cms;
+
+extern "C" size_t cms_consistency_workspace_bytes(const cms_consistency_desc* d) {
+    if (!d) return 0;
+    const Geo g = geo_of(d);
+    return LOSS_WS_HEAD + (size_t)std::max(fwd_blocks(g, 3), fused_tiles(g, 3)) * 3 * sizeof(float);
+}
+
+extern "C" int cms_consistency_fused_supported(const cms_consistency_desc* d) {
+    if (check_cons(d)) return 0;
+    return fused_tiles(geo_of(d), 3) > 0 ? 1 : 0;
+}
+
+extern "C" int cms_consistency_fwd_bwd(const cms_consistency_desc* d, float grad_unit, void* workspace, double* stats_out,
+                                       float* grad_l_stu, void* stream) {
+    return cons_fwd_bwd(d, grad_unit, 0.0f, 0.0f, workspace, stats_out, nullptr, nullptr, grad_l_stu, stream);
+}
+
+extern "C" int cms_consistency_fwd_bwd_finish(const cms_consistency_desc* d, float grad_unit, float ramp_val, float cons_weight,
+                                              void* workspace, double* stats_out, float* scalars_out, float* row_scale_out,
+                                              float* grad_l_stu, void* stream) {
+    CMS_REQUIRE(scalars_out, "consistency_fwd_bwd_finish: scalars_out NULL");
+    return cons_fwd_bwd(d, grad_unit, ramp_val, cons_weight, workspace, stats_out, scalars_out, row_scale_out, grad_l_stu, stream);
+}
+
+extern "C" size_t cms_loss_workspace_head_bytes(void) { return LOSS_WS_HEAD; }
+
+extern "C" int cms_loss_workspace_status(const void* workspace, void* stream) {
+    CMS_REQUIRE(workspace, "loss_workspace_status: NULL workspace");
+    unsigned head[2] = {0u, 0u};
+    hipError_t e = hipMemcpyAsync(head, workspace, sizeof(head), hipMemcpyDeviceToHost, (hipStream_t)stream);
+    if (e == hipSuccess) e = hipStreamSynchronize((hipStream_t)stream);
+    if (e != hipSuccess) {
+        set_error("cms_loss_workspace_status: %s", hipGetErrorString(e));
+        return CMS_ELAUNCH;
+    }
+    CMS_REQUIRE(head[0] == 0u && head[1] == 0u,
+                "loss workspace: a self-finishing launch found its ticket counter not zeroed (counter %u, status %u): zero the first "
+                "%zu bytes of the workspace once before its first launch", head[0], head[1], LOSS_WS_HEAD);
+    return CMS_OK;
 }
 
 extern "C" int cms_scale_by_scalar(float* x, long long n, const float* scalars, int index, float factor, void* stream) {
@@ -549,7 +637,7 @@
 extern "C" size_t cms_ce_workspace_bytes(const cms_ce_desc* d) {
     if (!d) return 0;
     const Geo g = geo_of(d);
-    return (size_t)std::max(fwd_blocks(g, 1), fused_tiles(g, 1)) * 2 * sizeof(float);
+    return LOSS_WS_HEAD + (size_t)std::max(fwd_blocks(g, 1), fused_tiles(g, 1)) * 2 * sizeof(float);
 }
 
 extern "C" int cms_ce_fused_supported(const cms_ce_desc* d) {
@@ -558,15 +646,13 @@
 }
 
 extern "C" int cms_ce_fwd_bwd(const cms_ce_desc* d, void* workspace, double* stats_out, float* grad_logits, void* stream) {
-    int rc = check_ce(d);
-    if (rc) return rc;
-    CMS_REQUIRE(workspace && stats_out && grad_logits, "ce_fwd_bwd: workspace / stats_out / grad NULL");
-    const CeArgs a = make_ce_args(d);
-    const int tiles = fused_tiles(a.g, 1);
-    CMS_REQUIRE(tiles > 0, "ce_fwd_bwd: not available for this geometry / mode (ask cms_ce_fused_supported)");
-    CMS_DISPATCH_C(d->c, launch_fused<2>(ce_fused_tiled_kernel<CT>, tiles, tile_lds_bytes(d->c, a.g.sy, a.g.sx, 1), (hipStream_t)stream,
-                                         (float*)workspace, stats_out, 0.0, -1, a, grad_logits));
-    return launch_status("cms_ce_fwd_bwd");
+    return ce_fwd_bwd(d, 0.0f, workspace, stats_out, nullptr, nullptr, grad_logits, stream);
+}
+
+extern "C" int cms_ce_fwd_bwd_finish(const cms_ce_desc* d, float loss_weight, void* workspace, double* stats_out, float* scalars_out,
+                                     float* row_scale_out, float* grad_logits, void* stream) {
+    CMS_REQUIRE(scalars_out, "ce_fwd_bwd_finish: scalars_out NULL");
+    return ce_fwd_bwd(d, loss_weight, workspace, stats_out, scalars_out, row_scale_out, grad_logits, stream);
 }
 
 extern "C" int cms_ce_fwd(const cms_ce_desc* d, void* workspace, double* stats_out, void* stream) {
diff --git a/cutmix-semisup-seg_amd/csrc/program.hip b/cutmix-semisup-seg_amd/csrc/program.hip
--- a/cutmix-semisup-seg_amd/csrc/program.hip
+++ b/cutmix-semisup-seg_amd/csrc/program.hip
@@ -130,7 +130,7 @@
     }
     case OP_ASPP_SPREAD: {
         const AsppOp& g = o.aspp;
-        return cms_aspp_spread_bwd(g.src, g.dst, g.d_dtype, g.tap_dy, g.tap_dx, g.n_taps, g.n, g.c, g.zc, g.h, g.w, s);
+        return cms_aspp_spread_bwd_scaled(g.src, g.bias, g.dst, g.d_dtype, g.tap_dy, g.tap_dx, g.n_taps, g.n, g.c, g.zc, g.h, g.w, s);
     }
     case OP_WGRAD:
         return o.f32 ? cms_conv_wgrad_f32(&o.wg, s) : cms_conv_wgrad(&o.wg, s);
@@ -301,6 +301,13 @@
                     group);
 }
 
+extern "C" int cms_program_add_aspp_spread_scaled(cms_program* p, const float* dlogits, const float* row_scale, void* d_nhwc,
+                                                  int d_dtype, const int* tap_dy, const int* tap_dx, int n_taps, int n, int c, int zc,
+                                                  int h, int w, int stream_idx, int group) {
+    return add_aspp(p, OP_ASPP_SPREAD, dlogits, row_scale, d_nhwc, d_dtype, tap_dy, tap_dx, n_taps, n, c, zc, h, w, stream_idx,
+                    group);
+}
+
 extern "C" int cms_program_add_bn(cms_program* p, const cms_bn_op* op, int stream_idx, int group) {
     CMS_REQUIRE(p && op, "program_add_bn: NULL pointer");
     CMS_REQUIRE(op->what >= CMS_BN_REDUCE && op->what <= CMS_BN_BWD_SUMS_TILES, "program_add_bn: unknown op %d", op->what);
diff --git a/cutmix-semisup-seg_amd/ops.py b/cutmix-semisup-seg_amd/ops.py
--- a/cutmix-semisup-seg_amd/ops.py
+++ b/cutmix-semisup-seg_amd/ops.py
@@ -135,6 +135,33 @@
     return torch.empty(max(int(fn['cms_{}_workspace_bytes'.format(name)](C.byref(d))), 16), dtype=torch.uint8, device=device)
 
 
+_FINISH_WS = {}
+
+
+def _finish_workspace(name, d, device):
+    nbytes = max(int(fn['cms_{}_workspace_bytes'.format(name)](C.byref(d))), 16)
+    key = (name, nbytes, str(device), int(torch.cuda.current_stream().cuda_stream))
+    ws = _FINISH_WS.get(key)
+    if ws is None:
+        ws = _FINISH_WS[key] = torch.zeros(nbytes, dtype=torch.uint8, device=device)
+    return ws
+
+
+def loss_workspace_check(ws):
+    check(fn['cms_loss_workspace_status'](_ptr(ws), _stream()), 'cms_loss_workspace_status')
+
+
+def _single_process(group):
+    import torch.distributed as dist
+    return not (dist.is_available() and dist.is_initialized() and dist.get_world_size(group) > 1)
+
+
+def _check_row_scale(who, row_scale, n):
+    if row_scale is not None and (row_scale.dtype != torch.float32 or row_scale.numel() != n or not row_scale.is_contiguous()
+                                  or not row_scale.is_cuda):
+        raise ValueError('{}: row_scale must be a contiguous f32 device tensor with one element per sample'.format(who))
+
+
 def _check_grad_out(who, grad_out, like):
     if grad_out.dtype != torch.float32 or tuple(grad_out.shape) != tuple(like.shape) or not grad_out.is_contiguous():
         raise ValueError('{}: grad_out must be a contiguous f32 tensor of the logits\' shape'.format(who))
@@ -207,24 +234,39 @@
 
 
 def consistency_fused(cfg, l_stu, l_tea0, l_tea1, out_size, grad_out, ranges=None, mask=None, um0=None, um1=None,
-                      ramp_val=1.0, cons_weight=1.0, group=None, sync_conf_rate=True):
+                      ramp_val=1.0, cons_weight=1.0, group=None, sync_conf_rate=True, row_scale=None, workspace=None):
     d, keep = _cons_prepare('consistency_fused', cfg, l_stu, l_tea0, l_tea1, out_size, ranges, mask, um0, um1, grad_out)
     l_stu, l_tea0, l_tea1, ranges, mask, um0, um1 = keep[:7]
+    _check_row_scale('consistency_fused', row_scale, int(d.n))
     if not fn['cms_consistency_fused_supported'](C.byref(d)):
         sc, cctx = consistency_forward(cfg, l_stu, l_tea0, l_tea1, out_size, ranges, mask, um0, um1, ramp_val, cons_weight, group,
                                        sync_conf_rate)
         consistency_backward(cctx, sc, grad_out)
+        if row_scale is not None:
+            row_scale.fill_(1.0)
         return sc
     dev = l_stu.device
-    ws = _workspace('consistency', d, dev)
     stats = torch.empty(4, dtype=torch.float64, device=dev)
     P = float(d.n) * float(d.H) * float(d.W)
     grad_unit = float(ramp_val) * float(cons_weight) / P
+    deferred = cfg.conf_thresh > 0.0 and not cfg.conf_per_pixel
+    if not (sync_conf_rate and cfg.conf_thresh > 0.0) or _single_process(group):
+        ws = workspace if workspace is not None else _finish_workspace('consistency', d, dev)
+        scalars = torch.empty(4, dtype=torch.float32, device=dev)
+        check(fn['cms_consistency_fwd_bwd_finish'](C.byref(d), grad_unit, float(ramp_val), float(cons_weight), _ptr(ws), _ptr(stats),
+                                                   _ptr(scalars), _ptr(row_scale) if row_scale is not None else None,
+                                                   _ptr(grad_out), _stream()), 'cms_consistency_fwd_bwd_finish')
+        if deferred and row_scale is None:
+            check(fn['cms_scale_by_scalar'](_ptr(grad_out), grad_out.numel(), _ptr(scalars), 1, 1.0, _stream()), 'cms_scale_by_scalar')
+        return scalars
+    ws = _workspace('consistency', d, dev)
     check(fn['cms_consistency_fwd_bwd'](C.byref(d), grad_unit, _ptr(ws), _ptr(stats), _ptr(grad_out), _stream()),
           'cms_consistency_fwd_bwd')
     scalars = _cons_scalars(stats, cfg, ramp_val, cons_weight, group, sync_conf_rate)
-    if cfg.conf_thresh > 0.0 and not cfg.conf_per_pixel:
+    if deferred:
         check(fn['cms_scale_by_scalar'](_ptr(grad_out), grad_out.numel(), _ptr(scalars), 1, 1.0, _stream()), 'cms_scale_by_scalar')
+    if row_scale is not None:
+        row_scale.fill_(1.0)
     return scalars
 
 
@@ -443,17 +485,31 @@
 
 
 def ce_fused(logits, labels, grad_out, out_size=None, ignore_index=255, align_corners=True, loss_weight=1.0, group=None,
-             sync_count=False):
+             sync_count=False, row_scale=None, workspace=None):
     d, logits, labels = _ce_prepare(logits, labels, out_size, ignore_index, align_corners, grad_out)
+    _check_row_scale('ce_fused', row_scale, int(d.n))
     if not fn['cms_ce_fused_supported'](C.byref(d)):
         sc, cctx = ce_forward(logits, labels, out_size, ignore_index, align_corners, loss_weight, group, sync_count)
         ce_backward(cctx, sc, grad_out)
+        if row_scale is not None:
+            row_scale.fill_(1.0)
         return sc
+    stats = torch.empty(2, dtype=torch.float64, device=logits.device)
+    if not sync_count or _single_process(group):
+        ws = workspace if workspace is not None else _finish_workspace('ce', d, logits.device)
+        scalars = torch.empty(2, dtype=torch.float32, device=logits.device)
+        check(fn['cms_ce_fwd_bwd_finish'](C.byref(d), float(loss_weight), _ptr(ws), _ptr(stats), _ptr(scalars),
+                                          _ptr(row_scale) if row_scale is not None else None, _ptr(grad_out), _stream()),
+              'cms_ce_fwd_bwd_finish')
+        if row_scale is None:
+            check(fn['cms_scale_by_scalar'](_ptr(grad_out), grad_out.numel(), _ptr(scalars), 1, 1.0, _stream()), 'cms_scale_by_scalar')
+        return scalars
     ws = _workspace('ce', d, logits.device)
-    stats = torch.empty(2, dtype=torch.float64, device=logits.device)
     check(fn['cms_ce_fwd_bwd'](C.byref(d), _ptr(ws), _ptr(stats), _ptr(grad_out), _stream()), 'cms_ce_fwd_bwd')
     scalars, _ = _ce_scalars(stats, loss_weight, group, sync_count)
     check(fn['cms_scale_by_scalar'](_ptr(grad_out), grad_out.numel(), _ptr(scalars), 1, 1.0, _stream()), 'cms_scale_by_scalar')
+    if row_scale is not None:
+        row_scale.fill_(1.0)
     return scalars
 
 
@@ -1421,6 +1477,10 @@
     def size(self):
         return int(fn['cms_program_size'](self.h))
 
+    @property
+    def dlg(self):
+        return self.dlg_in * self.row_scale.view(-1, 1, 1, 1)
+
     def mark(self, tag):
         self.marks.append((self.size(), tag))
 
@@ -1580,24 +1640,26 @@
     return out
 
 
-def aspp_spread_bwd(dlogits, taps, zc, dtype, out=None):
-    _need_cuda(dlogits, out)
+def aspp_spread_bwd(dlogits, taps, zc, dtype, out=None, row_scale=None):
+    _need_cuda(dlogits, out, row_scale)
     if dlogits.dtype != torch.float32 or not dlogits.is_contiguous():
         raise TypeError('aspp_spread_bwd: contiguous fp32 (N, C, h, w) gradient required')
     n, c, h, w = (int(v) for v in dlogits.shape)
+    _check_row_scale('aspp_spread_bwd', row_scale, n)
     if out is None:
         out = torch.empty((n, h, w, int(zc)), dtype=dtype, device=dlogits.device)
     dy, dx, nt = _tap_arrays(taps)
+    rs = _ptr(row_scale) if row_scale is not None else None
     if _REC is not None:
         prog = _REC[0]
-        idx = fn['cms_program_add_aspp_spread'](prog.h, _ptr(dlogits), _ptr(out), _dtype_code(out), dy, dx, nt, n, c,
-                                                int(zc), h, w, _rec_stream_index(), prog.group)
+        idx = fn['cms_program_add_aspp_spread_scaled'](prog.h, _ptr(dlogits), rs, _ptr(out), _dtype_code(out), dy, dx, nt, n, c,
+                                                       int(zc), h, w, _rec_stream_index(), prog.group)
         if idx < 0:
-            check(idx, 'cms_program_add_aspp_spread')
-        prog.keep += [dlogits, out]
+            check(idx, 'cms_program_add_aspp_spread_scaled')
+        prog.keep += [dlogits, out] + ([row_scale] if row_scale is not None else [])
         return out
-    check(fn['cms_aspp_spread_bwd'](_ptr(dlogits), _ptr(out), _dtype_code(out), dy, dx, nt, n, c, int(zc), h, w, _stream()),
-          'cms_aspp_spread_bwd')
+    check(fn['cms_aspp_spread_bwd_scaled'](_ptr(dlogits), rs, _ptr(out), _dtype_code(out), dy, dx, nt, n, c, int(zc), h, w, _stream()),
+          'cms_aspp_spread_bwd_scaled')
     return out
 
 
diff --git a/cutmix-semisup-seg_amd/step.py b/cutmix-semisup-seg_amd/step.py
--- a/cutmix-semisup-seg_amd/step.py
+++ b/cutmix-semisup-seg_amd/step.py
@@ -386,7 +386,16 @@
                 with torch.cuda.stream(side), torch.no_grad():
                     tea_lo = self.teacher.forward_lowres(x_tea)
             stu_lo = self.student.forward_lowres(x_stu)
-        grad_lo = torch.zeros(stu_lo.shape, dtype=torch.float32, device=stu_lo.device)
+        sex = self._student_executor()
+        row_scale = None
+        if (sex is not None and getattr(sex, 'use_programs', False) and hasattr(sex, 'dlogit_buffers')
+                and stu_lo.dtype == torch.float32 and stu_lo.is_contiguous() and stu_lo.grad_fn is not None
+                and type(stu_lo.grad_fn).__name__ in ('_BodyPairFnBackward', '_BodyFnBackward')):
+            grad_lo, row_scale = sex.dlogit_buffers(stu_lo.shape, stu_lo.device)
+            grad_lo.zero_()
+        else:
+            grad_lo = torch.zeros(stu_lo.shape, dtype=torch.float32, device=stu_lo.device)
+        rs_of = lambda a, b: None if row_scale is None else row_scale[a:b]
         lo_det = stu_lo.detach()
         split = use_unsup and side is not main
         if split:
@@ -402,7 +411,7 @@
                 t_off += 2 * n if cfg.mix else n
                 sc = ops.consistency_fused(cfg.cons, lo_det[s_off:s_off + n], l0, l1, out_size, grad_lo[s_off:s_off + n],
                                            ranges=ub.ranges, mask=ub.mask, um0=ub.um0, um1=ub.um1, ramp_val=ramp,
-                                           cons_weight=cfg.cons_weight, group=self.group)
+                                           cons_weight=cfg.cons_weight, group=self.group, row_scale=rs_of(s_off, s_off + n))
                 s_off += n
                 if split and isinstance(sc, torch.Tensor):
                     sc.record_stream(main)
@@ -410,8 +419,8 @@
         if split:
             with torch.cuda.stream(side):
                 consistency_branch()
-        ce_sc = ops.ce_fused(lo_det[:n_sup], sup_y, grad_lo[:n_sup], out_size, 255, self.align_corners, group=self.group)
-        sex = self._student_executor()
+        ce_sc = ops.ce_fused(lo_det[:n_sup], sup_y, grad_lo[:n_sup], out_size, 255, self.align_corners, group=self.group,
+                             row_scale=rs_of(0, n_sup))
         if split:
             if independent and groups is None and sex is not None and hasattr(sex, '_refresh_for_backward'):
                 sex._refresh_for_backward()
@@ -425,8 +434,12 @@
         if zev is not None:
             main.wait_event(zev)
         try:
+            if row_scale is not None:
+                sex.pending_row_scale = row_scale
             stu_lo.backward(grad_lo.to(stu_lo.dtype))
         finally:
+            if row_scale is not None:
+                sex.pending_row_scale = None
             if ex is not None:
                 ex.grad_hook = None
             if dex is not None:
diff --git a/include/cutmixseg.h b/include/cutmixseg.h
--- a/include/cutmixseg.h
+++ b/include/cutmixseg.h
@@ -76,6 +76,10 @@
 int cms_consistency_fwd_bwd(const cms_consistency_desc* d, float grad_unit, void* workspace, double* stats_out,
                             float* grad_l_stu, void* stream);
 int cms_scale_by_scalar(float* x, long long n, const float* scalars, int index, float factor, void* stream);
+int cms_consistency_fwd_bwd_finish(const cms_consistency_desc* d, float grad_unit, float ramp_val, float cons_weight, void* workspace,
+                                   double* stats_out, float* scalars_out, float* row_scale_out, float* grad_l_stu, void* stream);
+size_t cms_loss_workspace_head_bytes(void);
+int cms_loss_workspace_status(const void* workspace, void* stream);
 
 typedef struct cms_ce_desc {
     const float* logits;
@@ -91,6 +95,8 @@
 int cms_ce_bwd(const cms_ce_desc* d, const float* scalars, float* grad_logits, void* stream);
 int cms_ce_fused_supported(const cms_ce_desc* d);
 int cms_ce_fwd_bwd(const cms_ce_desc* d, void* workspace, double* stats_out, float* grad_logits, void* stream);
+int cms_ce_fwd_bwd_finish(const cms_ce_desc* d, float loss_weight, void* workspace, double* stats_out, float* scalars_out,
+                          float* row_scale_out, float* grad_logits, void* stream);
 int cms_loss_set_deterministic(int on);
 
 
@@ -387,6 +393,8 @@
                         int n, int c, int zc, int h, int w, void* stream);
 int cms_aspp_spread_bwd(const float* dlogits, void* d_nhwc, int d_dtype, const int* tap_dy, const int* tap_dx, int n_taps,
                         int n, int c, int zc, int h, int w, void* stream);
+int cms_aspp_spread_bwd_scaled(const float* dlogits, const float* row_scale, void* d_nhwc, int d_dtype, const int* tap_dy,
+                               const int* tap_dx, int n_taps, int n, int c, int zc, int h, int w, void* stream);
 
 int cms_stem_pack_weights(const void* w_khkwcoci, int w_dtype, float* w_packed, void* stream);
 int cms_stem_out_hw(int h, int w, int* ho, int* wo, int* hp, int* wp);
@@ -417,6 +425,9 @@
                                 const int* tap_dx, int n_taps, int n, int c, int zc, int h, int w, int stream_idx, int group);
 int cms_program_add_aspp_spread(cms_program* p, const float* dlogits, void* d_nhwc, int d_dtype, const int* tap_dy,
                                 const int* tap_dx, int n_taps, int n, int c, int zc, int h, int w, int stream_idx, int group);
+int cms_program_add_aspp_spread_scaled(cms_program* p, const float* dlogits, const float* row_scale, void* d_nhwc, int d_dtype,
+                                       const int* tap_dy, const int* tap_dx, int n_taps, int n, int c, int zc, int h, int w,
+                                       int stream_idx, int group);
 int cms_program_add_sync(cms_program* p, int from_stream, int to_stream, int group);
 int cms_program_sync_count(const cms_program* p);
 int cms_program_set_sync_flags(cms_program* p, int* flags_dev, int n_flags);
```

After: 642.2 images/sec. No clear change (-0.1%).
